# unknownue/puflow

Measured on AMD Instinct MI355X. Metric: patches/sec x4 2048->8192 (PU1K discrete, eval), higher is better.
Workload: dtype f32 (split-fp16 MFMA products, fp32 accumulate); 1 GPU; BASELINE configs[1]: PU1K discrete x4 inference, 32 x 2048-pt patches per GPU (fp32-parity mode); patches_per_gpu=32, total_batch=32, npoint=2048

## Files before the change

### include/puflow_hip.h

```cpp
#ifndef PUFLOW_HIP_H
#define PUFLOW_HIP_H

#ifdef __cplusplus
extern "C" {
#endif

#define PF_OK 0
#define PF_ERR_NULL (-1)
#define PF_ERR_SHAPE (-2)
#define PF_ERR_UNSUPPORTED (-3)
#define PF_ERR_LAUNCH (-4)
#define PF_ERR_WORKSPACE (-5)

int pf_version(void);
const char* pf_error_string(int code);

int pf_knn(const float* p1, const float* p2, int B, int N, int M, int K, int* idx_out, float* dist_out, void* stream);

int pf_nn1(const float* p1, const float* p2, int B, int N, int M, float* dist_out, int* idx_out, void* stream);

int pf_edgeconv(int cfg, const float* pq_or_xyz, const float* tab, const int* idx, const float* wfrag, float* out,
                int B, int N, void* stream);

int pf_edgeconv_tuned(int cfg, int variant, const float* pq_or_xyz, const float* tab, const int* idx,
                      const float* wfrag, float* out, int B, int N, void* stream);

int pf_edgeconv_pq(int unit, const float* pq_or_xyz, const int* idx, const float* wfrag, float* out, const float* w,
                   const long long* off, float* pq_next, int B, int N, int fuse, void* stream);

int pf_pq_gemm(int unit, const float* h, const float* w, const long long* off, float* pq_next, int T, void* stream);
int pf_cond(int unit, const float* h, const float* w, const long long* off, float* c, float* st, float* cp, int T,
            void* stream);
int pf_post(int unit, const float* h, const float* w, const long long* off, float* c, float* st, float* cp,
            float* pq_next, int T, void* stream);
int pf_cond_all(const float* const* h, const float* w, const long long* off, float* const* c, float* st, float* cp, int T,
                void* stream);

int pf_flow_fwd(const float* xyz, const float* cp, const float* st, const float* w, float* z, float* ld_pt, int T,
                void* stream);

int pf_flow_inv(const float* u, const float* cp, const float* st, const float* w, float* x, int T, int R, void* stream);

int pf_logp(const float* z, const float* ld_pt, float ld_const, int B, int N, float* ldj, float* lpsum, float* logp,
            void* stream);

long long pf_flow_fwd_logp_ws_floats(int B, int N);
int pf_flow_fwd_logp(const float* xyz, const float* cp, const float* st, const float* w, float* z, float* ld_pt,
                     float ld_const, int B, int N, float* ldj, float* lpsum, float* logp, float* ws, void* stream);

int pf_interp(const float* xyz, const float* z, const int* idx16, const float* w, const long long* off, float* u_out,
              int B, int N, int R, void* stream);

int pf_interp_weights(const float* xyz, const int* idx16, const float* w, const long long* off, float* aw_out, int B, int N,
                      void* stream);
int pf_flow_inv_interp(const float* aw, const float* z, const int* idx16, const float* cp, const float* st, const float* w,
                       float* x, int B, int N, int R, void* stream);

int pf_chamfer_fwd(const float* x, const float* y, int B, int N, int M, float* dist1, int* idx1, float* dist2,
                   int* idx2, float* per_sample, float* mean_sum, void* stream);

int pf_chamfer_bwd(const float* x, const float* y, const int* idx1, const int* idx2, const float* g1, const float* g2,
                   float* gx, float* gy, int B, int N, int M, void* stream);
int pf_chamfer_bwd_det(const float* x, const float* y, const int* idx1, const int* idx2, const float* g1, const float* g2,
                       float* gx, float* gy, int B, int N, int M, void* stream);

int pf_emd_forward(const float* xyz1, const float* xyz2, float* dist, int* assignment, float* price,
                   int* assignment_inv, int* bid, float* bid_increments, float* max_increments, int* unass_idx,
                   int* max_idx, float eps, int iters, int B, int n, void* stream);

int pf_emd_forward_ex(const float* xyz1, const float* xyz2, float* dist, int* assignment, float* price,
                      int* assignment_inv, int* bid, float* bid_increments, float* max_increments, int* unass_idx,
                      int* max_idx, float eps, int iters, int B, int n, int groups, unsigned* status, void* stream);

int pf_emd_backward(const float* xyz1, const float* xyz2, float* gradxyz, const float* graddist, const int* idx, int B,
                    int n, void* stream);


long long pf_gemm_ws_floats(int M, int N, int K);
int pf_gemm(const float* A, long long sam, long long sak, const float* B, long long sbk, long long sbn, float* C,
            long long ldc, const float* bias, int M, int N, int K, float* ws, long long ws_floats, void* stream);
int pf_gemm_reduce(const float* slabs, float* C, int M, int N, long long ldc, int nslab, void* stream);
int pf_gemm_ex(int arith, const float* A, long long sam, long long sak, const float* B, long long sbk, long long sbn, float* C,
               long long ldc, const float* bias, int M, int N, int K, float* ws, long long ws_floats, void* stream);

int pf_bn_chunks(long long R);
int pf_bn_lrelu_fwd(const float* x, long long R, int C, const float* gamma, const float* beta, float slope, float eps,
                    float momentum, float* run_mean, float* run_var, float* y, float* save, float* ws, void* stream);
int pf_bn_lrelu_bwd(const float* x, const float* dy, long long R, int C, const float* gamma, const float* beta, float slope,
                    const float* save, float* dx, float* dgamma, float* dbeta, float* ws, void* stream);
int pf_bn_colstat(const float* x, long long R, int C, const float* mean_in, float* out, float* ws, void* stream);
int pf_bn_apply_stats(const float* x, long long R, int C, const float* mean, const float* var_b, float unbias,
                      const float* gamma, const float* beta, float slope, float eps, float momentum, float* run_mean,
                      float* run_var, float* y, float* save, void* stream);
int pf_bn_bwd_sums(const float* x, const float* dy, long long R, int C, const float* gamma, const float* beta, float slope,
                   const float* save, float* sums, float* ws, void* stream);
int pf_bn_bwd_apply(const float* x, const float* dy, long long R, int C, const float* gamma, const float* beta, float slope,
                    const float* save, const float* means, float* dx, void* stream);
int pf_colsum(const float* g, long long R, int C, float* out, float* ws, void* stream);

int pf_act_fwd(const float* x, float slope, long long total, float* y, void* stream);
int pf_act_bwd(const float* y, const float* dy, float slope, long long total, float* dx, void* stream);

int pf_edge_feature_fwd(const float* x, const int* idx, int B, int N, int K, int C, float* out, void* stream);
int pf_edge_feature_bwd(const float* g, const int* idx, int B, int N, int K, int C, float* dx, void* stream);

int pf_maxpool_k_fwd(const float* y, long long T, int K, int C, float* out, int* arg, void* stream);
int pf_maxpool_k_bwd(const float* dy, const int* arg, long long T, int K, int C, float* dx, void* stream);

int pf_scatter_rows(const float* g, const int* idx, int B, int N, int K, int C, float* out, void* stream);
int pf_scatter_rows_det(const float* g, const int* csr_off, const int* csr_edge, long long T, int C, float* out, void* stream);
int pf_group_sum(const float* g, long long T, int R, int C, float* out, void* stream);

int pf_softmax_wsum_fwd(const float* w, int ldw, const float* zj, int K, int R, long long T, float* a, float* fz,
                        void* stream);
int pf_softmax_wsum_bwd(const float* a, const float* zj, const float* dfz, int K, int R, int ldw, long long T, float* dw,
                        float* dzj, void* stream);

int pf_actnorm_fwd(const float* x, const float* logs, const float* bias, int inv, long long R, float* y, void* stream);
int pf_actnorm_bwd(const float* x, const float* dy, const float* logs, const float* bias, int inv, long long R, float* dx,
                   float* glogs_rows, float* gbias_rows, void* stream);
int pf_couple_inject_fwd(const float* y, const float* o, const float* s, const float* t, int td, long long R, float* out,
                         void* stream);
int pf_couple_inject_bwd(const float* out, const float* dout, const float* s, int td, long long R, float* dy, float* do_,
                         float* ds, float* dt, void* stream);
int pf_inject_inv_fwd(const float* u, const float* s, const float* t, long long R, float* v, void* stream);
int pf_inject_inv_bwd(const float* u, const float* s, const float* dv, long long R, float* du, float* ds, float* dt,
                      void* stream);
int pf_couple_add(const float* v, const float* o, int td, long long R, float* out, void* stream);
int pf_slice_tail(const float* g, int td, long long R, float* o, void* stream);
int pf_batch_sum_fwd(const float* x, int B, long long M, int mode, float* out, void* stream);
int pf_batch_sum_bwd(const float* x, const float* g, int B, long long M, int mode, float* dx, void* stream);
int pf_dist_feature(const float* xyz, const int* idx, int B, int N, int K, float* out, void* stream);

#define PF_TRAIN_STAT_DOUBLES 4097
typedef struct PfEcTrain {
    int B, N, K, C, growth, nconv, odim, pooling;
    float slope, eps, momentum;
    const float* x;
    const int* idx;
    const float* W[9];
    const float* bias[9];
    const float* gamma[8]; const float* beta[8];
    float* run_mean[8]; float* run_var[8];
    float* Wpq;
    float* bpq;
    float* PQ;
    float* Y;
    float* aff;
    float* out;
    unsigned char* arg;
    const float* dout;
    float* dA;
    float* dPQ;
    float* coef;
    float* dWpq;
    float* dx;
    float* dW[9]; float* dbias[9]; float* dgamma[8]; float* dbeta[8];
    float* ws; long long ws_floats;
    double* stat;
    const int* csr_off; const int* csr_edge;
    int flags;
    unsigned* sync;
    int (*sync_cb)(void* user, double* sums, int n, void* stream);
    void* sync_user;
    double* sync_sums;
    float* ws_dw; long long ws_dw_floats;
    const float* dx_add;
} PfEcTrain;
#define PF_EC_PERSISTENT 1
#define PF_TRAIN_DETERMINISTIC 2
#define PF_EC_PREFOLDED 4
int pf_train_set_dw_stream(void* stream);
int pf_knn_csr(const int* idx, int B, int N, int K, int* off, int* edge, int* cnt, void* stream);
int pf_knn_csr_pair(const int* idx, int B, int N, int K, int K2, int* off, int* edge, int* off2, int* edge2, int* cnt, void* stream);

int pf_knn_csr_sort(const int* off, int* edge, int T, void* stream);
long long pf_ec_train_ws_floats(const PfEcTrain* p);
int pf_ec_train_fwd(const PfEcTrain* p, void* stream);
int pf_ec_train_fold_batch(const PfEcTrain* descs, int n, void* stream);
int pf_ec_train_bwd(const PfEcTrain* p, void* stream);

typedef struct PfBnMlpTrain {
    int rows, nl, kin0a, kin0b;
    int width[3];
    float slope, eps, momentum;
    const float* xa; const float* xb;
    const float* W[3]; const float* b[3];
// ... 287 lines not shown
```

### puflow_amd/_lib.py

```python
from __future__ import annotations

import ctypes
import os
from ctypes import c_char_p, c_double, c_float, c_int, c_longlong, c_ulonglong, c_void_p, POINTER

_HERE = os.path.dirname(os.path.abspath(__file__))
LIB_PATH = os.environ.get("PF_LIB_PATH", os.path.join(_HERE, "libpuflow_hip.so"))
_lib = None

class PfEcTrain(ctypes.Structure):
    _fields_ = [("B", c_int), ("N", c_int), ("K", c_int), ("C", c_int), ("growth", c_int), ("nconv", c_int), ("odim", c_int),
                ("pooling", c_int), ("slope", c_float), ("eps", c_float), ("momentum", c_float),
                ("x", c_void_p), ("idx", c_void_p), ("W", c_void_p * 9), ("bias", c_void_p * 9),
                ("gamma", c_void_p * 8), ("beta", c_void_p * 8), ("run_mean", c_void_p * 8), ("run_var", c_void_p * 8),
                ("Wpq", c_void_p), ("bpq", c_void_p), ("PQ", c_void_p), ("Y", c_void_p), ("aff", c_void_p), ("out", c_void_p),
                ("arg", c_void_p), ("dout", c_void_p), ("dA", c_void_p), ("dPQ", c_void_p), ("coef", c_void_p),
                ("dWpq", c_void_p), ("dx", c_void_p), ("dW", c_void_p * 9), ("dbias", c_void_p * 9),
                ("dgamma", c_void_p * 8), ("dbeta", c_void_p * 8), ("ws", c_void_p), ("ws_floats", c_longlong), ("stat", c_void_p), ("csr_off", c_void_p), ("csr_edge", c_void_p),
                ("flags", c_int), ("sync", c_void_p), ("sync_cb", c_void_p), ("sync_user", c_void_p), ("sync_sums", c_void_p),
                ("ws_dw", c_void_p), ("ws_dw_floats", c_longlong), ("dx_add", c_void_p)]


class PfBnMlpTrain(ctypes.Structure):
    _fields_ = [("rows", c_int), ("nl", c_int), ("kin0a", c_int), ("kin0b", c_int), ("width", c_int * 3),
                ("slope", c_float), ("eps", c_float), ("momentum", c_float), ("xa", c_void_p), ("xb", c_void_p),
                ("W", c_void_p * 3), ("b", c_void_p * 3), ("gamma", c_void_p * 2), ("beta", c_void_p * 2),
                ("run_mean", c_void_p * 2), ("run_var", c_void_p * 2), ("y", c_void_p * 3), ("aff", c_void_p * 2),
                ("dout", c_void_p), ("d", c_void_p * 2), ("coef", c_void_p * 2), ("dxa", c_void_p), ("dxb", c_void_p),
                ("dW", c_void_p * 3), ("db", c_void_p * 3), ("dgamma", c_void_p * 2), ("dbeta", c_void_p * 2),
                ("ws", c_void_p), ("ws_floats", c_longlong), ("stat", c_void_p),
                ("sync_cb", c_void_p), ("sync_user", c_void_p), ("sync_sums", c_void_p), ("flags", c_int)]


class PfMlpTrain(ctypes.Structure):
    _fields_ = [("rows", c_int), ("nl", c_int), ("td", c_int), ("ldy", c_int), ("cc", c_int), ("cdiv", c_int),
                ("width", c_int * 3), ("slope", c_float * 2), ("y", c_void_p), ("c", c_void_p),
                ("W", c_void_p * 3), ("b", c_void_p * 3), ("h", c_void_p * 2), ("out", c_void_p), ("dout", c_void_p),
                ("dz", c_void_p * 2), ("dy", c_void_p), ("dc", c_void_p), ("dW", c_void_p * 3), ("db", c_void_p * 3),
                ("ws", c_void_p), ("ws_floats", c_longlong), ("chunk", c_int), ("flags", c_int)]


_P8 = c_void_p * 8


class PfFlowChain(ctypes.Structure):
    _fields_ = [("nb", c_int), ("rows", c_int), ("R", c_int), ("inv", c_int), ("td", c_int * 8), ("cc", c_int * 8), ("n_ld", c_float),
                ("x", c_void_p), ("c", _P8), ("s", _P8), ("t", _P8), ("logs", _P8), ("bias", _P8), ("W", _P8),
                ("w0", _P8), ("w2", _P8), ("b2", _P8), ("w4", _P8), ("b4", _P8),
                ("pin", c_void_p), ("mid", c_void_p), ("o", c_void_p), ("h1", c_void_p), ("h2", c_void_p), ("out", c_void_p),
                ("ssum", c_void_p), ("ld", c_void_p), ("logp", c_void_p), ("Bsz", c_int), ("part", c_void_p), ("counter", c_void_p), ("img", c_void_p),
                ("dout", c_void_p), ("dssum", c_void_p), ("dld", c_void_p), ("dlogp", c_void_p), ("dx", c_void_p),
                ("dc", _P8), ("ds", _P8), ("dt", _P8), ("dz1", c_void_p), ("dz2", c_void_p), ("dob", c_void_p),
                ("dlogs", _P8), ("dbias", _P8), ("dW", _P8), ("dw0", _P8), ("dw2", _P8), ("db2", _P8), ("dw4", _P8), ("db4", _P8),
                ("ws", c_void_p), ("ws_floats", c_longlong), ("dev_descs", c_void_p), ("dz1s", c_void_p), ("img_ready", c_int)]


class PfPoissonPool(ctypes.Structure):
    _fields_ = [("off", c_int), ("s", c_int), ("m", c_int), ("out_off", c_int), ("R2", c_float), ("inv", c_float), ("lo", c_float),
                ("path", c_int)]


SIGNATURES = {
    "pf_version": (c_int, []),
    "pf_error_string": (c_char_p, [c_int]),
    "pf_knn": (c_int, [c_void_p, c_void_p, c_int, c_int, c_int, c_int, c_void_p, c_void_p, c_void_p]),
    "pf_nn1": (c_int, [c_void_p, c_void_p, c_int, c_int, c_int, c_void_p, c_void_p, c_void_p]),
    "pf_edgeconv": (c_int, [c_int, c_void_p, c_void_p, c_void_p, c_void_p, c_void_p, c_int, c_int, c_void_p]),
    "pf_edgeconv_tuned": (c_int, [c_int, c_int, c_void_p, c_void_p, c_void_p, c_void_p, c_void_p, c_int, c_int,
                                  c_void_p]),
    "pf_edgeconv_pq": (c_int, [c_int, c_void_p, c_void_p, c_void_p, c_void_p, c_void_p, POINTER(c_longlong), c_void_p, c_int, c_int, c_int,
                               c_void_p]),
    "pf_post": (c_int, [c_int, c_void_p, c_void_p, POINTER(c_longlong), c_void_p, c_void_p, c_void_p, c_void_p, c_int,
                        c_void_p]),
    "pf_pq_gemm": (c_int, [c_int, c_void_p, c_void_p, POINTER(c_longlong), c_void_p, c_int, c_void_p]),
    "pf_cond_all": (c_int, [POINTER(c_void_p), c_void_p, POINTER(c_longlong), POINTER(c_void_p), c_void_p, c_void_p, c_int, c_void_p]),
    "pf_cond": (c_int, [c_int, c_void_p, c_void_p, POINTER(c_longlong), c_void_p, c_void_p, c_void_p, c_int, c_void_p]),
    "pf_flow_fwd": (c_int, [c_void_p, c_void_p, c_void_p, c_void_p, c_void_p, c_void_p, c_int, c_void_p]),
    "pf_flow_inv": (c_int, [c_void_p, c_void_p, c_void_p, c_void_p, c_void_p, c_int, c_int, c_void_p]),
    "pf_flow_fwd_logp_ws_floats": (c_longlong, [c_int, c_int]),
    "pf_flow_fwd_logp": (c_int, [c_void_p, c_void_p, c_void_p, c_void_p, c_void_p, c_void_p, c_float, c_int, c_int, c_void_p, c_void_p,
                                 c_void_p, c_void_p, c_void_p]),
    "pf_logp": (c_int, [c_void_p, c_void_p, c_float, c_int, c_int, c_void_p, c_void_p, c_void_p, c_void_p]),
    "pf_interp": (c_int, [c_void_p, c_void_p, c_void_p, c_void_p, POINTER(c_longlong), c_void_p, c_int, c_int, c_int,
                          c_void_p]),
    "pf_interp_weights": (c_int, [c_void_p, c_void_p, c_void_p, POINTER(c_longlong), c_void_p, c_int, c_int, c_void_p]),
    "pf_flow_inv_interp": (c_int, [c_void_p, c_void_p, c_void_p, c_void_p, c_void_p, c_void_p, c_void_p, c_int, c_int, c_int, c_void_p]),
    "pf_chamfer_fwd": (c_int, [c_void_p, c_void_p, c_int, c_int, c_int, c_void_p, c_void_p, c_void_p, c_void_p, c_void_p,
                               c_void_p, c_void_p]),
    "pf_chamfer_bwd": (c_int, [c_void_p, c_void_p, c_void_p, c_void_p, c_void_p, c_void_p, c_void_p, c_void_p, c_int,
                               c_int, c_int, c_void_p]),
    "pf_chamfer_bwd_det": (c_int, [c_void_p, c_void_p, c_void_p, c_void_p, c_void_p, c_void_p, c_void_p, c_void_p, c_int,
                                   c_int, c_int, c_void_p]),
    "pf_emd_forward": (c_int, [c_void_p] * 11 + [c_float, c_int, c_int, c_int, c_void_p]),
    "pf_emd_forward_ex": (c_int, [c_void_p] * 11 + [c_float, c_int, c_int, c_int, c_int, c_void_p, c_void_p]),
    "pf_emd_backward": (c_int, [c_void_p, c_void_p, c_void_p, c_void_p, c_void_p, c_int, c_int, c_void_p]),
    "pf_gemm_ws_floats": (c_longlong, [c_int, c_int, c_int]),
    "pf_gemm": (c_int, [c_void_p, c_longlong, c_longlong, c_void_p, c_longlong, c_longlong, c_void_p, c_longlong, c_void_p,
                        c_int, c_int, c_int, c_void_p, c_longlong, c_void_p]),
    "pf_gemm_reduce": (c_int, [c_void_p, c_void_p, c_int, c_int, c_longlong, c_int, c_void_p]),
    "pf_gemm_ex": (c_int, [c_int, c_void_p, c_longlong, c_longlong, c_void_p, c_longlong, c_longlong, c_void_p, c_longlong, c_void_p,
                        c_int, c_int, c_int, c_void_p, c_longlong, c_void_p]),
    "pf_bn_chunks": (c_int, [c_longlong]),
    "pf_bn_lrelu_fwd": (c_int, [c_void_p, c_longlong, c_int, c_void_p, c_void_p, c_float, c_float, c_float, c_void_p,
                                c_void_p, c_void_p, c_void_p, c_void_p, c_void_p]),
    "pf_bn_lrelu_bwd": (c_int, [c_void_p, c_void_p, c_longlong, c_int, c_void_p, c_void_p, c_float, c_void_p, c_void_p,
                                c_void_p, c_void_p, c_void_p, c_void_p]),
    "pf_bn_colstat": (c_int, [c_void_p, c_longlong, c_int, c_void_p, c_void_p, c_void_p, c_void_p]),
    "pf_bn_apply_stats": (c_int, [c_void_p, c_longlong, c_int, c_void_p, c_void_p, c_float, c_void_p, c_void_p, c_float, c_float,
                                  c_float, c_void_p, c_void_p, c_void_p, c_void_p, c_void_p]),
    "pf_bn_bwd_sums": (c_int, [c_void_p, c_void_p, c_longlong, c_int, c_void_p, c_void_p, c_float, c_void_p, c_void_p, c_void_p,
                               c_void_p]),
    "pf_bn_bwd_apply": (c_int, [c_void_p, c_void_p, c_longlong, c_int, c_void_p, c_void_p, c_float, c_void_p, c_void_p, c_void_p,
                                c_void_p]),
    "pf_colsum": (c_int, [c_void_p, c_longlong, c_int, c_void_p, c_void_p, c_void_p]),
    "pf_act_fwd": (c_int, [c_void_p, c_float, c_longlong, c_void_p, c_void_p]),
    "pf_act_bwd": (c_int, [c_void_p, c_void_p, c_float, c_longlong, c_void_p, c_void_p]),
    "pf_edge_feature_fwd": (c_int, [c_void_p, c_void_p, c_int, c_int, c_int, c_int, c_void_p, c_void_p]),
    "pf_edge_feature_bwd": (c_int, [c_void_p, c_void_p, c_int, c_int, c_int, c_int, c_void_p, c_void_p]),
    "pf_maxpool_k_fwd": (c_int, [c_void_p, c_longlong, c_int, c_int, c_void_p, c_void_p, c_void_p]),
    "pf_maxpool_k_bwd": (c_int, [c_void_p, c_void_p, c_longlong, c_int, c_int, c_void_p, c_void_p]),
    "pf_scatter_rows": (c_int, [c_void_p, c_void_p, c_int, c_int, c_int, c_int, c_void_p, c_void_p]),
    "pf_scatter_rows_det": (c_int, [c_void_p, c_void_p, c_void_p, c_longlong, c_int, c_void_p, c_void_p]),
    "pf_group_sum": (c_int, [c_void_p, c_longlong, c_int, c_int, c_void_p, c_void_p]),
    "pf_softmax_wsum_fwd": (c_int, [c_void_p, c_int, c_void_p, c_int, c_int, c_longlong, c_void_p, c_void_p, c_void_p]),
    "pf_softmax_wsum_bwd": (c_int, [c_void_p, c_void_p, c_void_p, c_int, c_int, c_int, c_longlong, c_void_p, c_void_p,
                                    c_void_p]),
    "pf_actnorm_fwd": (c_int, [c_void_p, c_void_p, c_void_p, c_int, c_longlong, c_void_p, c_void_p]),
    "pf_actnorm_bwd": (c_int, [c_void_p, c_void_p, c_void_p, c_void_p, c_int, c_longlong, c_void_p, c_void_p, c_void_p, c_void_p]),
    "pf_couple_inject_fwd": (c_int, [c_void_p, c_void_p, c_void_p, c_void_p, c_int, c_longlong, c_void_p, c_void_p]),
    "pf_couple_inject_bwd": (c_int, [c_void_p, c_void_p, c_void_p, c_int, c_longlong, c_void_p, c_void_p, c_void_p, c_void_p,
                                     c_void_p]),
    "pf_inject_inv_fwd": (c_int, [c_void_p, c_void_p, c_void_p, c_longlong, c_void_p, c_void_p]),
    "pf_inject_inv_bwd": (c_int, [c_void_p, c_void_p, c_void_p, c_longlong, c_void_p, c_void_p, c_void_p, c_void_p]),
    "pf_couple_add": (c_int, [c_void_p, c_void_p, c_int, c_longlong, c_void_p, c_void_p]),
    "pf_slice_tail": (c_int, [c_void_p, c_int, c_longlong, c_void_p, c_void_p]),
    "pf_batch_sum_fwd": (c_int, [c_void_p, c_int, c_longlong, c_int, c_void_p, c_void_p]),
    "pf_batch_sum_bwd": (c_int, [c_void_p, c_void_p, c_int, c_longlong, c_int, c_void_p, c_void_p]),
    "pf_dist_feature": (c_int, [c_void_p, c_void_p, c_int, c_int, c_int, c_void_p, c_void_p]),
    "pf_fps": (c_int, [c_void_p, c_int, c_int, c_int, c_void_p, c_void_p, c_void_p]),
    "pf_fps_grouped": (c_int, [c_void_p, c_int, c_int, c_int, c_int, c_void_p, c_void_p, c_void_p]),
    "pf_fps_scratch_layout": (c_int, [c_int, POINTER(c_longlong), POINTER(c_longlong)]),
    "pf_fps_exchange_probe": (c_int, [c_int, c_int, c_void_p, c_void_p]),
    "pf_flow_params_fwd": (c_int, [c_void_p, c_void_p, c_float, c_void_p, c_void_p, c_void_p]),
    "pf_flow_params_bwd": (c_int, [c_void_p, c_void_p, c_void_p, c_float, c_void_p, c_void_p, c_void_p]),
    "pf_flow_affine_fwd": (c_int, [c_void_p, c_void_p, c_int, c_void_p, c_void_p, c_void_p, c_int, c_longlong, c_void_p, c_void_p]),
    "pf_flow_affine_bwd": (c_int, [c_void_p, c_void_p, c_int, c_void_p, c_void_p, c_void_p, c_int, c_longlong, c_void_p, c_void_p,
                                   c_void_p, c_void_p, c_void_p, c_void_p, c_void_p, c_void_p, c_void_p]),
    "pf_couple_inject2_fwd": (c_int, [c_void_p, c_void_p, c_void_p, c_void_p, c_int, c_longlong, c_void_p, c_void_p, c_void_p,
                                      c_void_p, c_void_p]),
    "pf_couple_inject2_bwd": (c_int, [c_void_p, c_void_p, c_void_p, c_void_p, c_int, c_longlong, c_void_p, c_void_p, c_void_p,
                                      c_void_p, c_void_p]),
    "pf_inject_inv2_fwd": (c_int, [c_void_p, c_void_p, c_void_p, c_int, c_longlong, c_void_p, c_void_p]),
    "pf_inject_inv2_bwd": (c_int, [c_void_p, c_void_p, c_void_p, c_int, c_longlong, c_void_p, c_void_p, c_void_p, c_void_p]),
    "pf_clip_adam": (c_int, [c_void_p, c_void_p, c_void_p, c_void_p, c_void_p, c_int, c_void_p, c_void_p, c_float, c_float, c_float,
                             c_float, c_void_p, c_void_p, c_void_p, c_void_p]),
    "pf_clip_adam_ptrs": (c_int, [c_void_p, c_void_p, c_void_p, c_void_p, c_void_p, c_int, c_void_p, c_void_p, c_float, c_float, c_float,
                             c_float, c_void_p, c_void_p, c_void_p, c_void_p]),
    "pf_mlp_train_ws_floats": (c_longlong, [c_void_p]),
    "pf_mlp_train_fwd": (c_int, [c_void_p, c_void_p]),
    "pf_mlp_train_bwd": (c_int, [c_void_p, c_void_p]),
    "pf_mlp_train_fwd_batch": (c_int, [c_void_p, c_int, c_void_p, c_void_p]),
    "pf_mlp_train_bwd_batch": (c_int, [c_void_p, c_int, c_void_p, c_void_p]),
    "pf_mlp_train_dw_batch": (c_int, [c_void_p, c_int, c_void_p, c_void_p]),
    "pf_flowchain_ws_floats": (c_longlong, [c_void_p]),
    "pf_flowchain_part_floats": (c_longlong, [c_void_p]),
    "pf_flowchain_img_floats": (c_longlong, [c_void_p]),
    "pf_flowchain_fwd": (c_int, [c_void_p, c_void_p]),
    "pf_flowchain_bwd": (c_int, [c_void_p, c_void_p]),
    "pf_interp_wsum_fwd": (c_int, [c_void_p, c_int, c_void_p, c_void_p, c_int, c_int, c_int, c_longlong, c_void_p, c_void_p, c_void_p]),
    "pf_interp_wsum_bwd": (c_int, [c_void_p, c_void_p, c_void_p, c_void_p, c_int, c_int, c_int, c_int, c_longlong, c_void_p, c_void_p,
                                   c_void_p]),
    "pf_interp_wsum_bwd_det": (c_int, [c_void_p, c_void_p, c_void_p, c_void_p, c_int, c_int, c_int, c_int, c_longlong, c_void_p, c_void_p,
                                       c_void_p, c_void_p, c_void_p]),
    "pf_emd_init": (c_int, [c_void_p, c_void_p, c_longlong, c_void_p]),
    "pf_pugan_loss_fwd": (c_int, [c_void_p, c_void_p, c_void_p, c_void_p, c_int, c_int, c_float, c_float, c_float, c_void_p, c_void_p]),
    "pf_pugan_loss_bwd": (c_int, [c_void_p, c_void_p, c_int, c_int, c_int, c_float, c_float, c_float, c_void_p, c_void_p, c_void_p,
                                  c_void_p, c_void_p, c_void_p, c_void_p]),
    "pf_pugan_grad": (c_int, [c_void_p] * 7 + [c_int] * 3 + [c_float] * 3 + [c_void_p] * 3),
    "pf_bnmlp_train_ws_floats": (c_longlong, [c_void_p]),
    "pf_bnmlp_train_fwd": (c_int, [c_void_p, c_void_p]),
    "pf_bnmlp_train_bwd": (c_int, [c_void_p, c_void_p]),
    "pf_train_set_dw_stream": (c_int, [c_void_p]),
    "pf_fold_wu_fwd": (c_int, [c_void_p] * 6 + [c_int] * 3 + [c_void_p] * 5),
    "pf_fold_wu_bwd": (c_int, [c_void_p] * 5 + [c_int] * 3 + [c_void_p] * 11),
    "pf_knn_csr": (c_int, [c_void_p, c_int, c_int, c_int, c_void_p, c_void_p, c_void_p, c_void_p]),
    "pf_knn_csr_pair": (c_int, [c_void_p, c_int, c_int, c_int, c_int, c_void_p, c_void_p, c_void_p, c_void_p, c_void_p, c_void_p]),
    "pf_knn_csr_sort": (c_int, [c_void_p, c_void_p, c_int, c_void_p]),
    "pf_ec_train_ws_floats": (c_longlong, [c_void_p]),
    "pf_ec_train_fwd": (c_int, [c_void_p, c_void_p]),
    "pf_ec_train_fold_batch": (c_int, [c_void_p, c_int, c_void_p]),
    "pf_ec_train_bwd": (c_int, [c_void_p, c_void_p]),
    "pf_cnf_init": (c_int, [c_void_p, c_void_p, c_int, c_void_p, c_void_p, c_void_p, c_void_p, c_void_p, c_double, c_double, c_double,
                            c_void_p, c_double, c_int, c_float, c_float, c_int, c_int, c_void_p, c_void_p]),
    "pf_cnf_context": (c_int, [c_void_p, c_int, c_void_p, c_void_p, c_float, c_void_p, c_int, c_void_p]),
    "pf_cnf_steps": (c_int, [c_void_p, c_void_p, c_void_p, c_void_p, c_void_p, c_void_p, c_void_p, c_void_p, c_void_p, c_float,
                             c_float, c_int, c_int, c_int, c_void_p, c_int, c_void_p]),
    "pf_knn_large": (c_int, [c_void_p, c_void_p, c_int, c_int, c_int, c_int, c_void_p, c_void_p, c_void_p]),
    "pf_normalize_pc": (c_int, [c_void_p, c_int, c_int, c_void_p, c_void_p, c_void_p, c_void_p]),
    "pf_normalize_pc_ragged": (c_int, [c_void_p, POINTER(c_int), c_int, c_void_p, c_void_p, c_void_p, c_void_p]),
    "pf_fps_ragged_layout": (c_int, [POINTER(c_int), c_int, c_int, POINTER(c_longlong), POINTER(c_int), POINTER(c_longlong),
                                     POINTER(c_longlong), POINTER(c_longlong)]),
    "pf_fps_ragged": (c_int, [c_void_p, POINTER(c_int), POINTER(c_int), c_int, c_int, c_void_p, c_void_p, c_void_p]),
    "pf_knn_large_ragged": (c_int, [c_void_p, c_void_p, POINTER(c_int), POINTER(c_int), c_int, c_int, c_void_p, c_void_p, c_void_p]),
    "pf_nn1_ragged": (c_int, [c_void_p, c_void_p, POINTER(c_int), POINTER(c_int), c_int, c_void_p, c_void_p, c_void_p]),
    "pf_format_xyz_bound": (c_longlong, [c_longlong, c_int]),
    "pf_format_xyz": (c_longlong, [c_void_p, c_longlong, c_int, c_void_p, c_longlong]),
    "pf_parse_xyz": (c_longlong, [c_void_p, c_longlong, c_void_p, c_longlong, POINTER(c_int)]),
    "pf_cnf_rhs": (c_int, [c_void_p, c_void_p, POINTER(c_float), c_int, c_float, c_float, c_float, c_void_p, c_void_p,
                           c_void_p, c_void_p, c_void_p, c_int, c_int, c_void_p]),
    "pf_cnf_rhs_vjp_workspace_bytes": (c_longlong, [c_int, c_int]),
    "pf_cnf_rhs_vjp": (c_int, [c_void_p, c_void_p, c_float, c_float, c_void_p, c_void_p, c_void_p, c_void_p, c_void_p, c_void_p,
                               c_int, c_int, c_void_p, c_void_p]),
    "pf_cnf_step": (c_int, [c_void_p, c_void_p, c_float, c_float, c_int, c_void_p, c_void_p, c_void_p, c_void_p, c_void_p,
                            c_void_p, c_float, c_float, c_int, c_int, c_void_p, c_void_p, c_void_p]),
    "pf_sum_n": (c_int, [POINTER(c_void_p), c_int, c_void_p, c_longlong, c_void_p]),
    "pf_copy_n": (c_int, [POINTER(c_void_p), POINTER(c_void_p), POINTER(c_longlong), c_int, c_void_p]),
    "pf_lincomb": (c_int, [POINTER(c_void_p), POINTER(c_float), c_int, c_void_p, c_longlong, c_void_p]),
    "pf_scaled_sumsq": (c_int, [c_void_p, c_void_p, c_void_p, c_void_p, c_void_p, POINTER(c_float), c_int, c_float, c_float,
                                c_float, c_longlong, c_void_p, c_void_p, c_void_p]),
    "pf_approxmatch_ws_floats": (c_longlong, [c_int, c_int, c_int, c_int]),
    "pf_approxmatch_emd": (c_int, [c_void_p, c_void_p, c_int, c_int, c_int, c_int, c_void_p, c_void_p, c_longlong, c_void_p]),
    "pf_point_mesh_ws_floats": (c_longlong, [c_int, c_int]),
    "pf_point_mesh_dist": (c_int, [c_void_p, c_int, c_void_p, c_int, c_void_p, c_int, c_void_p, c_void_p, c_void_p, c_longlong,
                                   c_void_p]),
    "pf_patch_batch": (c_int, [c_void_p, c_void_p, c_void_p, c_void_p, c_int, c_int, c_int, c_longlong, c_int, c_int, c_ulonglong,
                               c_ulonglong, c_int, c_float, c_float, c_float, c_float, c_float, c_void_p, c_void_p, c_void_p,
                               c_void_p, c_void_p, c_void_p, c_int, c_void_p, c_void_p]),
# ... 64 lines not shown
```

### puflow_amd/build.py

```python
from __future__ import annotations

import os
import subprocess
import sys

HERE = os.path.dirname(os.path.abspath(__file__))
CSRC = os.path.join(HERE, "csrc")
LIB = os.path.join(HERE, "libpuflow_hip.so")
SOURCES = ["api.hip", "knn.hip", "edgeconv.hip", "pointwise.hip", "flow.hip", "interp.hip", "chamfer.hip", "emd.hip", "train_ops.hip", "train_fused.hip", "train_ec_fwd.hip", "train_csr.hip", "train_bnmlp.hip", "train_mlp.hip", "train_flow.hip", "train_flowchain.hip", "train_glue.hip", "optim.hip", "patch_ops.hip", "cnf.hip", "cnf_bwd.hip", "xyz_io.hip", "eval_metrics.hip", "data_aug.hip", "eval_uniform.hip", "poisson.hip", "surface_reach.hip"]
FLAGS = ["--offload-arch=gfx950", "-O3", "-std=c++17", "-fPIC", "-ffp-contract=on", "-Wno-unused-result"]
EXTRA_FLAGS = {s: ["-fno-honor-nans", "-mllvm", "-amdgpu-mfma-vgpr-form=" + os.environ.get("PF_MFMA_VGPR_FORM", "1")] for s in ("edgeconv.hip", "pointwise.hip", "flow.hip", "interp.hip", "cnf.hip", "cnf_bwd.hip")}
EXTRA_FLAGS["edgeconv.hip"] = EXTRA_FLAGS["edgeconv.hip"] + ["-DPF_W2LDS_DEPTH=" + os.environ.get("PF_EC_W2LDS_DEPTH", "3")]
if os.environ.get("PF_INTERP_TRACKERS", "1") != "0":
    EXTRA_FLAGS["interp.hip"] = EXTRA_FLAGS["interp.hip"] + ["-mllvm", "-amdgpu-use-amdgpu-trackers=1"]


def _stale(target: str, deps) -> bool:
    if not os.path.exists(target):
        return True
    t = os.path.getmtime(target)
    return any(os.path.getmtime(d) > t for d in deps)


F16_SOURCES = ("edgeconv.hip", "pointwise.hip", "flow.hip", "interp.hip")
LIB_F16 = LIB.replace(".so", "_f16.so")


def build(force: bool = False, verbose: bool = True, defines=(), tag: str = "", only=None) -> str:
    hipcc = os.environ.get("HIPCC", "/opt/rocm/bin/hipcc")
    lib = LIB if not tag else LIB.replace(".so", f"_{tag}.so")
    srcs = [os.path.join(CSRC, s) for s in SOURCES if os.path.exists(os.path.join(CSRC, s))]
    hdrs = [os.path.join(CSRC, h) for h in os.listdir(CSRC) if h.endswith(".h")]
    hdrs.append(os.path.join(os.path.dirname(HERE), "include", "puflow_hip.h"))
    objdir = os.path.join(HERE, "build" + (f"_{tag}" if tag else ""))
    maindir = os.path.join(HERE, "build")
    os.makedirs(objdir, exist_ok=True)
    objs = []
    procs = []
    for s in srcs:
        base = os.path.basename(s)
        if only is not None and base not in only:
            objs.append(os.path.join(maindir, base.replace(".hip", ".o")))
            continue
        o = os.path.join(objdir, base.replace(".hip", ".o"))
        objs.append(o)
        if force or _stale(o, [s] + hdrs):
            cmd = [hipcc] + FLAGS + EXTRA_FLAGS.get(os.path.basename(s), []) + [f"-D{d}" for d in defines] + ["-c", s, "-o", o]
            if verbose:
                print(" ".join(cmd), flush=True)
            procs.append((s, subprocess.Popen(cmd)))
    for s, p in procs:
        if p.wait() != 0:
            raise RuntimeError(f"hipcc failed on {s}")
    if force or procs or _stale(lib, objs):
        cmd = [hipcc, "--offload-arch=gfx950", "-shared", "-fPIC", "-o", lib] + objs
        if verbose:
            print(" ".join(cmd), flush=True)
        subprocess.check_call(cmd)
    global _REFRESHING
    if not tag and not defines and not _REFRESHING:
        _REFRESHING = True
        try:
            _refresh_variants(lib, verbose)
        finally:
            _REFRESHING = False
    return lib


_REFRESHING = False


def _refresh_variants(lib: str, verbose: bool) -> None:
    pkg = os.path.dirname(lib)
    if os.path.exists(os.path.join(pkg, "libpuflow_hip_f16.so")) and _stale(os.path.join(pkg, "libpuflow_hip_f16.so"), [lib]):
        build_f16(verbose=verbose)
    if any(os.path.exists(os.path.join(pkg, f"libpuflow_hip_{t}.so")) and _stale(os.path.join(pkg, f"libpuflow_hip_{t}.so"), [lib])
           for t in ("bwdf32", "gradf32")):
        build_gradf32(verbose=verbose)


def build_f16(force: bool = False, verbose: bool = True) -> str:
    build(force=False, verbose=verbose)
    return build(force=force, verbose=verbose, defines=["PF_MMN_TERMS=1"], tag="f16", only=F16_SOURCES)


LIB_GRADF32 = LIB.replace(".so", "_gradf32.so")
GRADF32_DEFINES = ["PF_EC_BWDG_F32", "PF_EC_DW_F32", "PF_EC_FWD_F32"]
LIB_BWDF32 = LIB.replace(".so", "_bwdf32.so")
BWDF32_DEFINES = ["PF_EC_BWDG_F32", "PF_EC_DW_F32"]


def build_gradf32(force: bool = False, verbose: bool = True) -> str:
    build(force=False, verbose=verbose)
    build(force=force, verbose=verbose, defines=BWDF32_DEFINES, tag="bwdf32", only=("train_fused.hip",))
    return build(force=force, verbose=verbose, defines=GRADF32_DEFINES, tag="gradf32", only=("train_fused.hip", "train_ec_fwd.hip"))


if __name__ == "__main__":
    build(force="--force" in sys.argv)
    build_f16(force="--force" in sys.argv)
    build_gradf32(force="--force" in sys.argv)
    print(LIB)
    print(LIB_F16)
    print(LIB_GRADF32)
```

### puflow_amd/csrc/edgeconv.hip

```cpp
#include <hip/hip_runtime.h>
#include "pf_api_internal.h"
#include "pf_mfma.h"

namespace {

struct EcArgs {
    const float* pq;
    const float* xyz;
    const float* tab;
    const int* idx;
    const f4* wg;
    float* out;
    int T;
    int N;
    int chunk;
    int ntiles;
    const u4* pqf_w;
    const float* pqf_bias;
    const float* pqf_scales;
    float* pqf_out;
};

template <int ODIM>
__device__ __forceinline__ void pqf_stage(u4* hb, int ch, int pt, float v) {
    _Float16* h = reinterpret_cast<_Float16*>(hb);
    const int cp = ch >> 5, j = ((ch >> 4) & 1) * 4 + (ch & 3), slot = 16 * ((ch & 15) >> 2) + pt;
    const _Float16 hi = (_Float16)v;
    const _Float16 lo = (_Float16)(v - (float)hi);
    h[((cp * 2 + 0) * 64 + slot) * 8 + j] = hi;
    h[((cp * 2 + 1) * 64 + slot) * 8 + j] = lo;
}

constexpr int PQF_NT = 4;

template <int ODIM, int ROWS, int NW>
__device__ __forceinline__ void pqf_gemm(const EcArgs& a, const u4* hb, int nst, const int (&tpt)[PQF_NT], int wave_u, int lane) {
    constexpr int CP = ODIM / 32, RB = ROWS / 16 / NW;
    static_assert(ODIM % 32 == 0 && ROWS % (16 * NW) == 0, "rows split evenly over the waves");
    constexpr int OBW = NW <= 8 ? RB : 1;
    const int col = lane & 15, q = lane >> 4;
    const PfW2BufD<CP> ws(a.pqf_w, lane);
    const float inv = a.pqf_scales[6];
#pragma unroll
    for (int ob0 = 0; ob0 < RB; ob0 += OBW) {
        h8 wh[OBW][CP], wl[OBW][CP];
#pragma unroll
        for (int o = 0; o < OBW; ++o)
#pragma unroll
            for (int cp = 0; cp < CP; ++cp) {
                wh[o][cp] = ws.load((wave_u * RB + ob0 + o) * CP + cp, 0);
                wl[o][cp] = ws.load((wave_u * RB + ob0 + o) * CP + cp, 1);
            }
#pragma unroll
        for (int t = 0; t < PQF_NT; ++t) {
            if (t >= nst) break;
            const u4* hbt = hb + t * (CP * 2 * 64);
            f4 acc[OBW];
#pragma unroll
            for (int o = 0; o < OBW; ++o) acc[o] = pf_splat(0.f);
#pragma unroll
            for (int cp = 0; cp < CP; ++cp) {
                const h8 fh = __builtin_bit_cast(h8, hbt[(cp * 2 + 0) * 64 + lane]), fl = __builtin_bit_cast(h8, hbt[(cp * 2 + 1) * 64 + lane]);
#pragma unroll
                for (int o = 0; o < OBW; ++o) {
                    f4 x = acc[o];
                    if constexpr (PF_MMN_TERMS == 3) {
                        x = pf_mfma_f16(wh[o][cp], fl, x);
                        x = pf_mfma_f16(wl[o][cp], fh, x);
                    }
                    x = pf_mfma_f16(wh[o][cp], fh, x);
                    acc[o] = x;
                }
            }
            const int pt = tpt[t] + col;
            if (pt < a.T) {
#pragma unroll
                for (int o = 0; o < OBW; ++o) {
                    const f4 bias = *reinterpret_cast<const f4*>(a.pqf_bias + (wave_u * RB + ob0 + o) * 16 + 4 * q);
                    f4 v;
#pragma unroll
                    for (int r = 0; r < 4; ++r) v[r] = fmaf(acc[o][r], inv, bias[r]);
                    *reinterpret_cast<f4*>(a.pqf_out + (size_t)pt * ROWS + (wave_u * RB + ob0 + o) * 16 + 4 * q) = v;
                }
            }
        }
    }
}

struct PqfState {
    int nst = 0;
    int tpt[PQF_NT] = {0, 0, 0, 0};
    __device__ __forceinline__ void push(int pt0) {
#pragma unroll
        for (int k = 0; k < PQF_NT; ++k) tpt[k] = k == nst ? pt0 : tpt[k];
        ++nst;
    }
};

template <int GB, int NCONV, int ODIM, bool C3, int P, int NW>
__global__ __launch_bounds__(NW * 64) void edgeconv_kernel(EcArgs a) {
    constexpr int G = GB * 16;
    constexpr int S = G * NCONV + ODIM;
    constexpr int NF = GB * NCONV;
    constexpr int OBO = ODIM / 16;
    constexpr int OCH = 2;
    static_assert(OBO <= 16 && OBO % OCH == 0, "pooled store uses one lane column per output block");
    const int lane = threadIdx.x & 63, wave = threadIdx.x >> 6;
    const int col = lane & 15, q = lane >> 4;

    constexpr int NWF = GB * GB * (NCONV * (NCONV - 1) / 2) + OBO * NF;
    __shared__ f4 wlds[NWF * 64];
    pf_stage_lds(wlds, a.wg, NWF * 64);
    __syncthreads();
    const PfWLds ws{wlds, lane};

    for (int v = blockIdx.x; v < 8 * a.chunk; v += gridDim.x) {
        const int tile = pf_xcd_tile(v, a.chunk);
        if (tile >= a.ntiles) continue;
        const int pt0 = (tile * NW + wave) * P;

        int gi[P], gj[P];
        float xi[P][3], xj[P][3];
#pragma unroll
        for (int p = 0; p < P; ++p) {
            int g = pt0 + p;
            g = g < a.T ? g : a.T - 1;
            gi[p] = g;
            const int b = g / a.N;
            gj[p] = b * a.N + a.idx[(size_t)g * 16 + col];
            if constexpr (C3) {
#pragma unroll
                for (int c = 0; c < 3; ++c) {
                    xi[p][c] = a.xyz[(size_t)gi[p] * 3 + c];
                    xj[p][c] = a.xyz[(size_t)gj[p] * 3 + c];
                }
            }
        }

        auto init = [&](int p, int off) -> f4 {
            if constexpr (C3) {
                f4 r;
#pragma unroll
                for (int k = 0; k < 4; ++k) {
                    const f4* t = reinterpret_cast<const f4*>(a.tab + (size_t)(off + k) * 8);
                    const f4 t0 = t[0], t1 = t[1];
                    float s = t1.z;
                    s = fmaf(t0.x, xi[p][0], s); s = fmaf(t0.y, xi[p][1], s); s = fmaf(t0.z, xi[p][2], s);
                    s = fmaf(t0.w, xj[p][0], s); s = fmaf(t1.x, xj[p][1], s); s = fmaf(t1.y, xj[p][2], s);
                    r[k] = s;
                }
                return r;
            } else {
                const f4 pv = *reinterpret_cast<const f4*>(a.pq + (size_t)gi[p] * (2 * S) + off);
                const f4 qv = *reinterpret_cast<const f4*>(a.pq + (size_t)gj[p] * (2 * S) + S + off);
                return pv + qv;
            }
        };

        constexpr int NI = GB > OCH ? GB : OCH;
        f4 ini[2][P][NI];
        auto load_init = [&](auto nbc, int row0, f4 (&dst)[P][NI]) {
            constexpr int NB = decltype(nbc)::value;
#pragma unroll
            for (int ob = 0; ob < NB; ++ob)
#pragma unroll
                for (int p = 0; p < P; ++p) dst[p][ob] = init(p, row0 + ob * 16 + 4 * q);
        };
        using IGB = std::integral_constant<int, GB>;
        using IOC = std::integral_constant<int, OCH>;
        load_init(IGB{}, 0, ini[0]);
        if constexpr (NCONV > 1) load_init(IGB{}, G, ini[1]); else load_init(IOC{}, G * NCONV, ini[1]);

        f4 feat[P][NF];
#pragma unroll
        for (int ob = 0; ob < GB; ++ob)
#pragma unroll
            for (int p = 0; p < P; ++p) feat[p][ob] = pf_lrelu(ini[0][p][ob], 0.05f);

        pf_static_for<1, NCONV>([&](auto tc) {
            constexpr int t = decltype(tc)::value;
            if constexpr (t + 1 < NCONV) load_init(IGB{}, G * (t + 1), ini[(t + 1) & 1]);
            else load_init(IOC{}, G * NCONV, ini[(t + 1) & 1]);
            f4 acc[P][GB];
#pragma unroll
            for (int ob = 0; ob < GB; ++ob)
#pragma unroll
                for (int p = 0; p < P; ++p) acc[p][ob] = ini[t & 1][p][ob];
            pf_mm<GB, GB * t, GB * t>(ws, GB * GB * (t * (t - 1) / 2), feat, 0, acc, 0);
#pragma unroll
            for (int ob = 0; ob < GB; ++ob)
#pragma unroll
                for (int p = 0; p < P; ++p) feat[p][GB * t + ob] = pf_lrelu(acc[p][ob], 0.05f);
        });

        constexpr int FO = GB * GB * (NCONV * (NCONV - 1) / 2);
        f4 sel[P];
#pragma unroll
        for (int p = 0; p < P; ++p) sel[p] = pf_splat(0.f);
        pf_static_for<0, OBO / OCH>([&](auto cc) {
            constexpr int c = decltype(cc)::value;
            constexpr int ob0 = c * OCH;
            constexpr int st = NCONV + c;
            if constexpr (c + 1 < OBO / OCH) load_init(IOC{}, G * NCONV + (ob0 + OCH) * 16, ini[(st + 1) & 1]);
            f4 acc[P][OCH];
#pragma unroll
            for (int o = 0; o < OCH; ++o)
#pragma unroll
                for (int p = 0; p < P; ++p) acc[p][o] = ini[st & 1][p][o];
            pf_mm<OCH, NF, NF>(ws, FO + ob0 * NF, feat, 0, acc, 0);
#pragma unroll
            for (int o = 0; o < OCH; ++o)
#pragma unroll
                for (int p = 0; p < P; ++p) {
                    f4 m;
#pragma unroll
                    for (int r = 0; r < 4; ++r) m[r] = pf_rowmax16(acc[p][o][r]);
                    if (col == ob0 + o) sel[p] = m;
                }
        });
#pragma unroll
        for (int p = 0; p < P; ++p)
            if (col < OBO && pt0 + p < a.T)
                *reinterpret_cast<f4*>(a.out + (size_t)gi[p] * ODIM + col * 16 + 4 * q) = sel[p];
    }
}

struct EcWConst {
    static constexpr int DEPTH = 2;
    int lane;
    __device__ __forceinline__ h8 load(int frag, int split) const {
        const _Float16 x = (_Float16)(float)((lane + frag + split) & 7);
        return (h8){x, x, x, x, x, x, x, x};
    }
};

constexpr float EC4_OUT_INV = 1.f / 256.f;

template <int P, int NW, int DBG = 0, bool PQF = false>
__global__ __launch_bounds__(NW * 64) void edgeconv4_kernel(EcArgs a) {
    static_assert(!PQF || NW * P == 16, "the fused P|Q GEMM takes a workgroup tile of 16 points as one MFMA column tile");
    constexpr int NCONV = 4, G = 32, S = 256, OBO = 8, OCH = 2, ODIM = 128;
    constexpr int NWF = 2 * (NCONV * (NCONV - 1) / 2) + OBO * NCONV;
    constexpr int ROWB = 2 * S * 4;
    const int lane = threadIdx.x & 63, wave = threadIdx.x >> 6;
    const int col = lane & 15, q = lane >> 4;
    __shared__ u4 wlds[NWF * 2 * 64];
    __shared__ f4 plds[NW * P][64];
    __shared__ u4 hb[PQF ? PQF_NT * (ODIM / 32) * 2 * 64 : 1];
    PqfState pqf;
    pf_stage_lds(wlds, reinterpret_cast<const u4*>(a.wg), NWF * 2 * 64);
    __syncthreads();
    const PfW2Lds ws_lds{wlds, lane};
    const auto ws = [&] { if constexpr ((DBG & 4) != 0) return EcWConst{lane}; else return ws_lds; }();
    const __amdgpu_buffer_rsrc_t rs = __builtin_amdgcn_make_buffer_rsrc(const_cast<float*>(a.pq), 0, 0x7fffffff, 0x00020000);
    const int blkq = ((q & 1) << 1) | (q >> 1);

    const int vend = 8 * a.chunk;
    auto next_valid = [&](int v) { while (v < vend && pf_xcd_tile(v, a.chunk) >= a.ntiles) v += gridDim.x; return v; };
    struct Pre { int g[P]; int jc[P]; int4 j4[P]; f4 prow[P]; };
    auto fetch = [&](int v, Pre& n) {
        const int pt0 = (pf_xcd_tile(v < vend ? v : blockIdx.x, a.chunk) * NW + wave) * P;
#pragma unroll
        for (int p = 0; p < P; ++p) {
            int g = pt0 + p;
            g = g < a.T ? g : a.T - 1;
            g = __builtin_amdgcn_readfirstlane(g);
            n.g[p] = g;
            n.jc[p] = a.idx[(size_t)g * 16 + col];
            n.j4[p] = *reinterpret_cast<const int4*>(a.idx + (size_t)g * 16 + 4 * q);
            n.prow[p] = __builtin_bit_cast(f4, __builtin_amdgcn_raw_buffer_load_b128(rs, lane * 16, g * ROWB, 0));
        }
    };
    int v = next_valid(blockIdx.x);
    Pre cur;
    if (v < vend) fetch(v, cur);
    while (v < vend) {
        const int pt0 = (pf_xcd_tile(v, a.chunk) * NW + wave) * P;
        const int vn = next_valid(v + gridDim.x);
        int vQ[P];
        int vO[P][4];
        int gout[P];
#pragma unroll
        for (int p = 0; p < P; ++p) {
            const int g = cur.g[p];
            const int bN = (g / a.N) * a.N;
            gout[p] = g;
            plds[wave * P + p][lane] = cur.prow[p];
            vQ[p] = (bN + cur.jc[p]) * ROWB + (S + 4 * q) * 4;
            vO[p][0] = (bN + cur.j4[p].x) * ROWB + (S + G * NCONV + col) * 4;
            vO[p][1] = (bN + cur.j4[p].y) * ROWB + (S + G * NCONV + col) * 4;
            vO[p][2] = (bN + cur.j4[p].z) * ROWB + (S + G * NCONV + col) * 4;
            vO[p][3] = (bN + cur.j4[p].w) * ROWB + (S + G * NCONV + col) * 4;
        }
        fetch(vn, cur);
        auto load_g = [&](int t, f4 (&dst)[P][2]) {
#pragma unroll
            for (int ob = 0; ob < 2; ++ob)
#pragma unroll
                for (int p = 0; p < P; ++p) {
                    const int off = (G * t + 16 * ob) * 4;
                    if constexpr (DBG & 1) { dst[p][ob] = pf_splat((float)(off + vQ[p]) * 1e-9f); continue; }
                    dst[p][ob] = __builtin_bit_cast(f4, __builtin_amdgcn_raw_buffer_load_b128(rs, vQ[p], off, 0));
                }
        };
        auto p_g = [&](int p, int t, int ob) -> f4 { return plds[wave * P + p][(G * t + 16 * ob) / 4 + q]; };
        auto load_o = [&](int ob0, f4 (&dst)[P][2]) {
#pragma unroll
            for (int o = 0; o < OCH; ++o)
#pragma unroll
                for (int p = 0; p < P; ++p)
#pragma unroll
                    for (int r = 0; r < 4; ++r) {
                        if constexpr (DBG & 1) { dst[p][o][r] = (float)(vO[p][r] + ob0 + o) * 1e-9f; continue; }
                        dst[p][o][r] = __builtin_bit_cast(float, __builtin_amdgcn_raw_buffer_load_b32(rs, vO[p][r], (ob0 + o) * 64, 0));
                    }
        };
        f4 ini[2][P][2];
        load_g(0, ini[0]);
        load_g(1, ini[1]);
        PfPairN feat[P][NCONV];
#pragma unroll
        for (int p = 0; p < P; ++p)
            feat[p][0] = pf_pairn(pf_lrelu(ini[0][p][0] + p_g(p, 0, 0), 0.05f), pf_lrelu(ini[0][p][1] + p_g(p, 0, 1), 0.05f));
        pf_static_for<1, NCONV>([&](auto tc) {
            constexpr int t = decltype(tc)::value;
            if constexpr (t + 1 < NCONV) load_g(t + 1, ini[(t + 1) & 1]); else load_o(0, ini[(t + 1) & 1]);
            f4 acc[P][2];
#pragma unroll
            for (int ob = 0; ob < 2; ++ob)
#pragma unroll
                for (int p = 0; p < P; ++p) acc[p][ob] = ini[t & 1][p][ob] + p_g(p, t, ob);
            if constexpr (!(DBG & 2)) pf_mmn<false, 2, t, t>(ws, 2 * (t * (t - 1) / 2), feat, acc);
#pragma unroll
            for (int p = 0; p < P; ++p) {
                if constexpr (DBG & 8) { feat[p][t] = feat[p][0]; feat[p][t].h[0] += (_Float16)acc[p][0].x; continue; }
                feat[p][t] = pf_pairn(pf_lrelu(acc[p][0], 0.05f), pf_lrelu(acc[p][1], 0.05f));
            }
        });
        constexpr int FO = 2 * (NCONV * (NCONV - 1) / 2);
        float m[P][OBO];
        pf_static_for<0, OBO / OCH>([&](auto cc) {
            constexpr int c = decltype(cc)::value;
            constexpr int ob0 = c * OCH;
            constexpr int st = NCONV + c;
            if constexpr (c + 1 < OBO / OCH) load_o(ob0 + OCH, ini[(st + 1) & 1]);
            f4 acc[P][OCH];
#pragma unroll
            for (int o = 0; o < OCH; ++o)
#pragma unroll
                for (int p = 0; p < P; ++p) acc[p][o] = ini[st & 1][p][o];
            if constexpr (!(DBG & 2)) pf_mmn<true, OCH, NCONV, NCONV>(ws, FO + ob0 * NCONV, feat, acc);
#pragma unroll
            for (int o = 0; o < OCH; ++o)
#pragma unroll
                for (int p = 0; p < P; ++p)
                    m[p][ob0 + o] = fmaxf(fmaxf(acc[p][o].x, acc[p][o].y), fmaxf(acc[p][o].z, acc[p][o].w));
        });
#pragma unroll
        for (int p = 0; p < P; ++p) {
            const float o0 = pf_rsmax16(pf_rsmax32(m[p][0], m[p][1]), pf_rsmax32(m[p][2], m[p][3]));
            const float o1 = pf_rsmax16(pf_rsmax32(m[p][4], m[p][5]), pf_rsmax32(m[p][6], m[p][7]));
            const int ch = 16 * blkq + col;
            const float* pr = reinterpret_cast<const float*>(plds[wave * P + p]);
            const float p0 = pr[G * NCONV + ch], p1 = pr[G * NCONV + 64 + ch];
            const float h0 = fmaf(o0, EC4_OUT_INV, p0), h1 = fmaf(o1, EC4_OUT_INV, p1);
            if (pt0 + p < a.T) {
                float* o = a.out + (size_t)gout[p] * ODIM + ch;
                o[0] = h0;
                o[64] = h1;
            }
            if constexpr (PQF) {
                u4* hbt = hb + pqf.nst * ((ODIM / 32) * 2 * 64);
                pqf_stage<ODIM>(hbt, ch, wave * P + p, h0);
                pqf_stage<ODIM>(hbt, ch + 64, wave * P + p, h1);
            }
        }
        if constexpr (PQF) {
            pqf.push(pf_xcd_tile(v, a.chunk) * NW * P);
            if (pqf.nst == PQF_NT || vn >= vend) {
                __syncthreads();
                pqf_gemm<ODIM, 2 * S, NW>(a, hb, pqf.nst, pqf.tpt, __builtin_amdgcn_readfirstlane(wave), lane);
                __syncthreads();
                pqf.nst = 0;
            }
        }
        v = vn;
    }
}

template <int P, int NW, int DBG = 0, bool PQF = false>
int launch4(const EcArgs& a0, hipStream_t s) {
    EcArgs a = a0;
    a.ntiles = (a.T + NW * P - 1) / (NW * P);
    a.chunk = (a.ntiles + 7) / 8;
    int grid = 8 * a.chunk;
    if (grid > 256) grid = 256;
    hipLaunchKernelGGL((edgeconv4_kernel<P, NW, DBG, PQF>), dim3(grid), dim3(NW * 64), 0, s, a);
    return pf_last_launch_status();
}

template <int ODIM, bool C3, int P, int NW, bool PQF = false>
__global__ __launch_bounds__(NW * 64) void edgeconv1n_kernel(EcArgs a) {
    static_assert(!PQF || NW * P == 16, "the fused P|Q GEMM takes a workgroup tile of 16 points as one MFMA column tile");
    constexpr int NCONV = 4, S = 16 * NCONV + ODIM, SB = S / 16, OBO = ODIM / 16;
    constexpr int PQ_ROWS = ODIM == 32 ? 256 : 512;
    constexpr int FO = 4, FT = FO + OBO * 2, NWF = FT + (C3 ? SB : 0);
    constexpr int ROWB = 2 * S * 4;
    static_assert(OBO == 2 || OBO == 4, "reduce-scatter below is written for 2 or 4 output blocks");
    const int lane = threadIdx.x & 63, wave = threadIdx.x >> 6;
    const int col = lane & 15, q = lane >> 4;
    __shared__ u4 wlds[NWF * 128];
    __shared__ float plds[C3 ? 1 : NW * P][C3 ? 1 : S];
    __shared__ u4 hb[PQF ? PQF_NT * (ODIM / 32) * 2 * 64 : 1];
    PqfState pqf;
    pf_stage_lds(wlds, reinterpret_cast<const u4*>(a.wg), NWF * 128);
    __syncthreads();
    const PfW2Lds ws{wlds, lane};
    const __amdgpu_buffer_rsrc_t rs = __builtin_amdgcn_make_buffer_rsrc(const_cast<float*>(C3 ? a.xyz : a.pq), 0, 0x7fffffff, 0x00020000);

    for (int v = blockIdx.x; v < 8 * a.chunk; v += gridDim.x) {
        const int tile = pf_xcd_tile(v, a.chunk);
        if (tile >= a.ntiles) continue;
        const int pt0 = (tile * NW + wave) * P;
        int gi[P], vQ[P], vO[P][4];
        PfPairN e[P][1];
#pragma unroll
        for (int p = 0; p < P; ++p) {
            int g = pt0 + p;
            g = g < a.T ? g : a.T - 1;
            g = __builtin_amdgcn_readfirstlane(g);
            gi[p] = g;
            const int bN = (g / a.N) * a.N;
            const int jc = bN + a.idx[(size_t)g * 16 + col];
            if constexpr (C3) {
                float xi[3], xj[3];
#pragma unroll
                for (int c = 0; c < 3; ++c) {
                    xi[c] = a.xyz[(size_t)g * 3 + c];
                    xj[c] = a.xyz[(size_t)jc * 3 + c];
                }
                const f4 z4 = pf_splat(0.f);
                const f4 e0 = {xi[0], xi[1], xi[2], xj[0]}, e1 = {xj[1], xj[2], 0.f, 1.f};
                e[p][0] = pf_pairn(q == 0 ? e0 : z4, q == 0 ? e1 : z4);
            } else {
                const int4 j4 = *reinterpret_cast<const int4*>(a.idx + (size_t)g * 16 + 4 * q);
                vQ[p] = jc * ROWB + (S + 4 * q) * 4;
                vO[p][0] = (bN + j4.x) * ROWB + (S + 16 * NCONV + col) * 4;
                vO[p][1] = (bN + j4.y) * ROWB + (S + 16 * NCONV + col) * 4;
                vO[p][2] = (bN + j4.z) * ROWB + (S + 16 * NCONV + col) * 4;
                vO[p][3] = (bN + j4.w) * ROWB + (S + 16 * NCONV + col) * 4;
                if (lane * 2 < S) {
                    typedef float f2 __attribute__((ext_vector_type(2)));
                    const f2 pv = *reinterpret_cast<const f2*>(a.pq + (size_t)g * (2 * S) + lane * 2);
                    *reinterpret_cast<f2*>(&plds[wave * P + p][lane * 2]) = pv;
                }
            }
        }
        f4 pre[P][NCONV];
        f4 outi[P][OBO];
        if constexpr (C3) {
#pragma unroll
            for (int p = 0; p < P; ++p) {
#pragma unroll
                for (int b = 0; b < NCONV; ++b) pre[p][b] = pf_splat(0.f);
#pragma unroll
                for (int b = 0; b < OBO; ++b) outi[p][b] = pf_splat(0.f);
            }
            pf_mmn<false, NCONV, 1, 1>(ws, FT, e, pre);
            pf_mmn<true, OBO, 1, 1>(ws, FT + NCONV, e, outi);
        } else {
#pragma unroll
            for (int b = 0; b < NCONV; ++b)
#pragma unroll
                for (int p = 0; p < P; ++p)
                    pre[p][b] = __builtin_bit_cast(f4, __builtin_amdgcn_raw_buffer_load_b128(rs, vQ[p], b * 64, 0));
#pragma unroll
            for (int b = 0; b < OBO; ++b)
#pragma unroll
                for (int p = 0; p < P; ++p)
#pragma unroll
                    for (int r = 0; r < 4; ++r)
                        outi[p][b][r] = __builtin_bit_cast(float, __builtin_amdgcn_raw_buffer_load_b32(rs, vO[p][r], b * 64, 0));
#pragma unroll
            for (int b = 0; b < NCONV; ++b)
#pragma unroll
                for (int p = 0; p < P; ++p) pre[p][b] += *reinterpret_cast<const f4*>(&plds[wave * P + p][16 * b + 4 * q]);
        }

        PfPairN fp[P][2];
        f4 last[P];
#pragma unroll
        for (int p = 0; p < P; ++p) {
            last[p] = pf_lrelu(pre[p][0], 0.05f);
            fp[p][0] = pf_pairn(last[p], pf_splat(0.f));
        }
        pf_static_for<1, NCONV>([&](auto tc) {
            constexpr int t = decltype(tc)::value;
            constexpr int CPT = (t + 1) / 2, F0 = (t / 2) * ((t + 1) / 2);
            f4 acc[P][1];
#pragma unroll
            for (int p = 0; p < P; ++p) acc[p][0] = pre[p][t];
            pf_mmn<false, 1, CPT, CPT>(ws, F0, fp, acc);
#pragma unroll
            for (int p = 0; p < P; ++p) {
                const f4 f = pf_lrelu(acc[p][0], 0.05f);
                if constexpr (t % 2 == 1) fp[p][t / 2] = pf_pairn(last[p], f);
                else fp[p][t / 2] = pf_pairn(f, pf_splat(0.f));
                last[p] = f;
            }
        });
        pf_mmn<true, OBO, 2, 2>(ws, FO, fp, outi);
#pragma unroll
        for (int p = 0; p < P; ++p) {
            float m[OBO];
#pragma unroll
            for (int b = 0; b < OBO; ++b) m[b] = fmaxf(fmaxf(outi[p][b].x, outi[p][b].y), fmaxf(outi[p][b].z, outi[p][b].w));
            float o;
            int ch;
            if constexpr (OBO == 4) {
                o = pf_rsmax16(pf_rsmax32(m[0], m[1]), pf_rsmax32(m[2], m[3]));
                ch = 16 * (((q & 1) << 1) | (q >> 1)) + col;
            } else {
                const float n = pf_rsmax32(m[0], m[1]);
                o = pf_rsmax16(n, n);
                ch = 16 * (q >> 1) + col;
            }
            float pv = 0.f;
            if constexpr (!C3) pv = plds[wave * P + p][16 * NCONV + ch];
            const float hv = fmaf(o, EC4_OUT_INV, pv);
            if (pt0 + p < a.T && (OBO == 4 || (q & 1) == 0))
                a.out[(size_t)gi[p] * ODIM + ch] = hv;
            if constexpr (PQF) {
                if (OBO == 4 || (q & 1) == 0) pqf_stage<ODIM>(hb + pqf.nst * ((ODIM / 32) * 2 * 64), ch, wave * P + p, hv);
            }
        }
        if constexpr (PQF) {
            pqf.push(tile * NW * P);
            if (pqf.nst == PQF_NT) {
                __syncthreads();
                pqf_gemm<ODIM, PQ_ROWS, NW>(a, hb, pqf.nst, pqf.tpt, __builtin_amdgcn_readfirstlane(wave), lane);
                __syncthreads();
                pqf.nst = 0;
            }
        }
    }
    if constexpr (PQF) {
        if (pqf.nst > 0) {
            __syncthreads();
            pqf_gemm<ODIM, PQ_ROWS, NW>(a, hb, pqf.nst, pqf.tpt, __builtin_amdgcn_readfirstlane(wave), lane);
        }
    }
}

template <int ODIM, bool C3, int P, int NW, bool PQF = false>
int launch1n(const EcArgs& a0, hipStream_t s) {
    EcArgs a = a0;
    a.ntiles = (a.T + NW * P - 1) / (NW * P);
    a.chunk = (a.ntiles + 7) / 8;
    int grid = 8 * a.chunk;
    const int cap = 256 * (32 / NW);
    if (grid > cap) grid = cap;
    hipLaunchKernelGGL((edgeconv1n_kernel<ODIM, C3, P, NW, PQF>), dim3(grid), dim3(NW * 64), 0, s, a);
    return pf_last_launch_status();
}

template <int ODIM, bool C3>
int launch1n_v(const EcArgs& a, hipStream_t s, int variant) {
    switch (variant) {
        case 1: return launch1n<ODIM, C3, 2, 8>(a, s);
#ifdef PF_TUNING_VARIANTS
        case 0: return launch1n<ODIM, C3, 1, 8>(a, s);
        case 2: return launch1n<ODIM, C3, 1, 16>(a, s);
        case 3: return launch1n<ODIM, C3, 2, 4>(a, s);
#endif
        default: return PF_ERR_UNSUPPORTED;
    }
}

template <int GB, int NCONV, int ODIM, bool C3, int P, int NW>
int launch_v(const EcArgs& a0, hipStream_t s) {
    EcArgs a = a0;
    a.ntiles = (a.T + NW * P - 1) / (NW * P);
    a.chunk = (a.ntiles + 7) / 8;
    constexpr int NF = GB * NCONV;
    constexpr int lds = (GB * GB * (NCONV * (NCONV - 1) / 2) + (ODIM / 16) * NF) * 1024;
    int per_cu = (160 * 1024) / lds;
    const int by_waves = 32 / NW;
    if (per_cu > by_waves) per_cu = by_waves;
    if (per_cu < 1) per_cu = 1;
    int grid = 8 * a.chunk;
    const int cap = 256 * per_cu;
    if (grid > cap) grid = cap;
    hipLaunchKernelGGL((edgeconv_kernel<GB, NCONV, ODIM, C3, P, NW>), dim3(grid), dim3(NW * 64), 0, s, a);
    return pf_last_launch_status();
}

template <int GB, int NCONV, int ODIM, bool C3>
int launch(const EcArgs& a, hipStream_t s, int variant) {
    constexpr int BEST = ODIM == 32 ? 0 : (ODIM == 64 ? 2 : 3);
    if (variant == BEST) {
        if constexpr (BEST == 0) return launch_v<GB, NCONV, ODIM, C3, 2, 8>(a, s);
        else if constexpr (BEST == 2) return launch_v<GB, NCONV, ODIM, C3, 1, 8>(a, s);
        else return launch_v<GB, NCONV, ODIM, C3, 1, 16>(a, s);
    }
#ifdef PF_TUNING_VARIANTS
    switch (variant) {
        case 0: return launch_v<GB, NCONV, ODIM, C3, 2, 8>(a, s);
        case 1: return launch_v<GB, NCONV, ODIM, C3, 2, 4>(a, s);
        case 2: return launch_v<GB, NCONV, ODIM, C3, 1, 8>(a, s);
        case 3: return launch_v<GB, NCONV, ODIM, C3, 1, 16>(a, s);
        default: break;
    }
#endif
    return PF_ERR_UNSUPPORTED;
}

}

extern "C" int pf_edgeconv_tuned(int cfg, int variant, const float* pq_or_xyz, const float* tab, const int* idx,
                                 const float* wfrag, float* out, int B, int N, void* stream) {
    if (!pq_or_xyz || !idx || !wfrag || !out) return PF_ERR_NULL;
    if (B <= 0 || N < 16 || (long long)B * N > (1ll << 30)) return PF_ERR_SHAPE;
    EcArgs a{};
    a.idx = idx; a.wg = reinterpret_cast<const f4*>(wfrag); a.out = out; a.T = B * N; a.N = N;
    hipStream_t s = (hipStream_t)stream;
    switch (cfg) {
        case 0:
            if (!tab) return PF_ERR_NULL;
            a.xyz = pq_or_xyz; a.tab = tab;
            return launch<1, 4, 32, true>(a, s, variant);
        case 1: a.pq = pq_or_xyz; return launch<1, 4, 64, false>(a, s, variant);
        case 2: a.pq = pq_or_xyz; return launch<2, 4, 128, false>(a, s, variant);
        case 7:
            {
                const long long maxT = 0x7fffffffll / 2048;
                if (N > maxT) return PF_ERR_UNSUPPORTED;
                const int Bc = (int)(maxT / N);
                for (int b0 = 0; b0 < B; b0 += Bc) {
                    const int nb = B - b0 < Bc ? B - b0 : Bc;
                    EcArgs c = a;
                    c.pq = pq_or_xyz + (size_t)b0 * N * 512; c.idx = idx + (size_t)b0 * N * 16; c.out = out + (size_t)b0 * N * 128;
                    c.T = nb * N;
                    int rc;
                    switch (variant) {
                        case 0: rc = launch4<1, 16>(c, s); break;
#ifdef PF_TUNING_VARIANTS
                        case 1: rc = launch4<2, 8>(c, s); break;
                        case 2: rc = launch4<1, 8>(c, s); break;
                        case 3: rc = launch4<2, 4>(c, s); break;
                        case 8: rc = launch4<1, 16, 1>(c, s); break;
                        case 9: rc = launch4<1, 16, 2>(c, s); break;
                        case 10: rc = launch4<1, 16, 4>(c, s); break;
                        case 11: rc = launch4<1, 16, 5>(c, s); break;
                        case 12: rc = launch4<1, 16, 3>(c, s); break;
                        case 13: rc = launch4<1, 16, 6>(c, s); break;
                        case 14: rc = launch4<1, 16, 13>(c, s); break;
#endif
                        default: return PF_ERR_UNSUPPORTED;
                    }
                    if (rc != PF_OK) return rc;
// ... 47 lines not shown
```

### puflow_amd/csrc/flow.hip

```cpp
#include <hip/hip_runtime.h>
#include "pf_api_internal.h"
#include "pf_mfma.h"
#include "pf_wave.h"

#ifndef PF_FLOW_NW
#define PF_FLOW_NW 16
#endif
#ifndef PF_FLOW_NW_FWD
#define PF_FLOW_NW_FWD 16
#endif

namespace {

constexpr int FLOW_REC = 5360;
constexpr float LOG2PI_F = 1.8378770664093453f;

struct FlowArgs {
    const float* in;
    const float* cp;
    const float* st;
    const float* w;
    float* out;
    float* ld_pt;
    int T;
    int R;
    int rows;
    int ntiles;
    float* part;
    unsigned* counter;
    float* ldj; float* lps; float* logp;
    float ld_const;
    int B, N;
    const float* aw;
    const float* z;
    const int* idx;
};

struct FlowCond { f4 cp[4]; f4 s0, s1; };

__device__ __forceinline__ FlowCond flow_cond(const float* __restrict__ cp, const float* __restrict__ st, int T, int u,
                                              int pt, int q) {
    FlowCond c;
    const float* cr = cp + ((size_t)u * T + pt) * 64 + 4 * q;
#pragma unroll
    for (int cb = 0; cb < 4; ++cb) c.cp[cb] = *reinterpret_cast<const f4*>(cr + cb * 16);
    const float* sr = st + ((size_t)u * T + pt) * 8;
    c.s0 = *reinterpret_cast<const f4*>(sr);
    c.s1 = *reinterpret_cast<const f4*>(sr + 4);
    return c;
}

template <int TD>
__device__ __forceinline__ void coupling_net(const float* rec , int lane, int q, const FlowCond& c,
                                             const float (&h1)[2], float (&o)[2]) {
    PfPairN hp[1][2];
    const float i2 = rec[5352], i4 = rec[5353];
    {
        f4 hid[4];
#pragma unroll
        for (int cb = 0; cb < 4; ++cb) {
            const f4 wa = *reinterpret_cast<const f4*>(rec + 5200 + (cb * 16 + 4 * q) * 2);
            const f4 wb = *reinterpret_cast<const f4*>(rec + 5200 + (cb * 16 + 4 * q) * 2 + 4);
            f4 v = c.cp[cb];
            v.x = fmaf(wa.x, h1[0], v.x); v.y = fmaf(wa.z, h1[0], v.y);
            v.z = fmaf(wb.x, h1[0], v.z); v.w = fmaf(wb.z, h1[0], v.w);
            if (TD == 2) {
                v.x = fmaf(wa.y, h1[1], v.x); v.y = fmaf(wa.w, h1[1], v.y);
                v.z = fmaf(wb.y, h1[1], v.z); v.w = fmaf(wb.w, h1[1], v.w);
            }
            hid[cb] = pf_lrelu(v, 0.01f);
        }
        hp[0][0] = pf_pairn(hid[0], hid[1]);
        hp[0][1] = pf_pairn(hid[2], hid[3]);
    }
    const PfW2Lds ws{reinterpret_cast<const u4*>(rec), lane};
    f4 h2[1][4];
#pragma unroll
    for (int ob = 0; ob < 4; ++ob) h2[0][ob] = pf_bias(rec + 5120, ob, q);
    pf_mmn<false, 4, 2, 2>(ws, 0, hp, h2);
    hp[0][0] = pf_pairn(pf_lrelu(h2[0][0] * i2, 0.01f), pf_lrelu(h2[0][1] * i2, 0.01f));
    hp[0][1] = pf_pairn(pf_lrelu(h2[0][2] * i2, 0.01f), pf_lrelu(h2[0][3] * i2, 0.01f));
    f4 acc[1][1];
    acc[0][0] = *reinterpret_cast<const f4*>(rec + 5184 + 4 * q);
    pf_mmn<false, 1, 2, 2>(ws, 8, hp, acc);
    o[0] = acc[0][0].x * i4; o[1] = acc[0][0].y * i4;
}

template <bool INV, int NW>
__global__ __launch_bounds__(NW * 64) void flow_kernel(FlowArgs a) {
    const int lane = threadIdx.x & 63, wave = threadIdx.x >> 6;
    const int col = lane & 15, q = lane >> 4;
    __shared__ f4 wl[6 * FLOW_REC / 4];
    pf_stage_lds(wl, reinterpret_cast<const f4*>(a.w), 6 * FLOW_REC / 4);
    __syncthreads();
    const float* wlf = reinterpret_cast<const float*>(wl);

    for (int tile = blockIdx.x; tile < a.ntiles; tile += gridDim.x) {
        const int g = (tile * NW + wave) * 16 + col;
        const bool ok = g < a.rows;
        const int row = ok ? g : a.rows - 1;
        const int pt = row / a.R;
        float v[3], ld = 0.f;
        if (INV && a.aw) {
            const int r = row - pt * a.R, bN = (pt / a.N) * a.N;
            const int4 j0 = *reinterpret_cast<const int4*>(a.idx + (size_t)pt * 16), j1 = *reinterpret_cast<const int4*>(a.idx + (size_t)pt * 16 + 4);
            const int jj[8] = {j0.x, j0.y, j0.z, j0.w, j1.x, j1.y, j1.z, j1.w};
            float sk[8][3];
#pragma unroll
            for (int k = 0; k < 8; ++k) {
                const float wk = a.aw[((size_t)pt * 8 + k) * 4 + r];
                const float* zz = a.z + (size_t)(bN + jj[k]) * 3;
#pragma unroll
                for (int c = 0; c < 3; ++c) sk[k][c] = __fmul_rn(wk, zz[c]);
            }
#pragma unroll
            for (int c = 0; c < 3; ++c)
                v[c] = __fadd_rn(__fadd_rn(__fadd_rn(sk[0][c], sk[1][c]), __fadd_rn(sk[2][c], sk[3][c])),
                                 __fadd_rn(__fadd_rn(sk[4][c], sk[5][c]), __fadd_rn(sk[6][c], sk[7][c])));
        } else {
#pragma unroll
            for (int c = 0; c < 3; ++c) v[c] = a.in[(size_t)row * 3 + c];
        }
        FlowCond cn = flow_cond(a.cp, a.st, a.T, INV ? 5 : 0, pt, q);

        pf_static_for<0, 6>([&](auto uc) {
            constexpr int i = decltype(uc)::value;
            constexpr int u = INV ? 5 - i : i;
            constexpr int TD = (u % 2 == 0) ? 1 : 2;
            const float* rec = wlf + u * FLOW_REC;
            const float* fc = rec + 5328;
            const FlowCond c = cn;
            if constexpr (i < 5) cn = flow_cond(a.cp, a.st, a.T, INV ? u - 1 : u + 1, pt, q);
            __builtin_amdgcn_sched_barrier(0);
            const float s[3] = {c.s0.x, c.s0.y, c.s0.z}, t[3] = {c.s0.w, c.s1.x, c.s1.y};
            float h1[2], o[2];
            if constexpr (!INV) {
                const float x0 = v[0], x1 = v[1], x2 = v[2];
#pragma unroll
                for (int k = 0; k < 3; ++k)
                    v[k] = fmaf(fc[3 * k + 2], x2, fmaf(fc[3 * k + 1], x1, fmaf(fc[3 * k], x0, fc[9 + k])));
                h1[0] = v[0]; h1[1] = v[1];
                coupling_net<TD>(rec, lane, q, c, h1, o);
                if (TD == 1) { v[1] -= o[0]; v[2] -= o[1]; } else { v[2] -= o[0]; }
                const float y0 = v[2], y1 = v[1], y2 = v[0];
                v[0] = (y0 - t[0]) * expf(-s[0]);
                v[1] = (y1 - t[1]) * expf(-s[1]);
                v[2] = (y2 - t[2]) * expf(-s[2]);
                ld -= (s[0] + s[1]) + s[2];
            } else {
                const float y0 = fmaf(v[0], expf(s[0]), t[0]);
                const float y1 = fmaf(v[1], expf(s[1]), t[1]);
                const float y2 = fmaf(v[2], expf(s[2]), t[2]);
                v[0] = y2; v[1] = y1; v[2] = y0;
                h1[0] = v[0]; h1[1] = v[1];
                coupling_net<TD>(rec, lane, q, c, h1, o);
                if (TD == 1) { v[1] += o[0]; v[2] += o[1]; } else { v[2] += o[0]; }
                const float x0 = v[0], x1 = v[1], x2 = v[2];
#pragma unroll
                for (int k = 0; k < 3; ++k)
                    v[k] = fmaf(fc[12 + 3 * k + 2], x2, fmaf(fc[12 + 3 * k + 1], x1, fmaf(fc[12 + 3 * k], x0, fc[21 + k])));
            }
        });

        if (ok && q == 0) {
            a.out[(size_t)row * 3 + 0] = v[0];
            a.out[(size_t)row * 3 + 1] = v[1];
            a.out[(size_t)row * 3 + 2] = v[2];
            if (!INV) a.ld_pt[row] = ld;
        }
        if constexpr (!INV) {
            if (a.part) {
                float sl = ld;
                float sz = -0.5f * (v[0] * v[0] + LOG2PI_F) + -0.5f * (v[1] * v[1] + LOG2PI_F) + -0.5f * (v[2] * v[2] + LOG2PI_F);
                sl += __shfl_xor(sl, 1); sz += __shfl_xor(sz, 1);
                sl += __shfl_xor(sl, 2); sz += __shfl_xor(sz, 2);
                sl += __shfl_xor(sl, 4); sz += __shfl_xor(sz, 4);
                sl += __shfl_xor(sl, 8); sz += __shfl_xor(sz, 8);
                if (ok && lane == 0) {
                    const int wt = g >> 4;
                    PF_ST(a.part + wt, sl);
                    PF_ST(a.part + (a.rows >> 4) + wt, sz);
                }
            }
        }
    }
    if constexpr (!INV) {
        if (!a.part) return;
        __shared__ float sa[NW * 64];
        __shared__ int is_last;
        asm volatile("s_waitcnt vmcnt(0)" ::: "memory");
        __syncthreads();
        if (threadIdx.x == 0) is_last = atomicAdd(a.counter, 1u) == gridDim.x - 1 ? 1 : 0;
        __syncthreads();
        if (!is_last) return;
        const int tid = threadIdx.x;
        const int per = a.N >> 4, half = a.rows >> 4;
        for (int b = wave; b < a.B; b += NW) {
            float accl = 0.f, accz = 0.f;
            for (int i = lane; i < per; i += 64) {
                accl += PF_LD(a.part + b * per + i);
                accz += PF_LD(a.part + half + b * per + i);
            }
            accl = pf_xor_sum<32, 1>(accl); accz = pf_xor_sum<32, 1>(accz);
            if (lane == 0) {
                const float l = accl + a.ld_const * (float)a.N;
                a.ldj[b] = l;
                a.lps[b] = accz + l;
                if (b < NW * 64) sa[b] = accz + l;
            }
        }
        __syncthreads();
        float tot = 0.f;
        if (tid == 0)
            for (int b = 0; b < a.B; ++b) tot += b < NW * 64 ? sa[b] : a.lps[b];
        if (tid == 0) {
            *a.logp = -tot / (float)a.B;
            PF_ST(a.counter, 0u);
        }
    }
}

template <bool INV, int NW>
int launch_nw(FlowArgs a, hipStream_t s) {
    a.ntiles = (a.rows + NW * 16 - 1) / (NW * 16);
    const int grid = a.ntiles < 256 ? a.ntiles : 256;
    hipLaunchKernelGGL((flow_kernel<INV, NW>), dim3(grid), dim3(NW * 64), 0, s, a);
    return pf_last_launch_status();
}

template <bool INV>
int launch(FlowArgs a, hipStream_t s) {
    constexpr int NWMAX = INV ? PF_FLOW_NW : PF_FLOW_NW_FWD;
    const int wt = (a.rows + 15) / 16;
    if (wt >= 200 * NWMAX) return launch_nw<INV, NWMAX>(a, s);
// ... 95 lines not shown
```

### puflow_amd/csrc/interp.hip

```cpp
#include <hip/hip_runtime.h>
#include "pf_api_internal.h"
#include "pf_mfma.h"
#include "pf_wave.h"

#ifndef PF_INTERP_P
#define PF_INTERP_P 1
#endif
#ifndef PF_INTERP_NW
#define PF_INTERP_NW 12
#endif

namespace {

struct InterpArgs {
    const float* xyz;
    const float* z;
    const int* idx;
    const float* w;
    long long off[15];
    float* u;
    float* aw;
    int T, N, ntiles, R;
    int per;
    int contiguous;
};

template <int P, int NW, bool BIG = false>
__global__ __launch_bounds__(NW * 64) void interp_kernel(InterpArgs a) {
    constexpr int R = 4;
    const int lane = threadIdx.x & 63, wave = threadIdx.x >> 6;
    const int col = lane & 15, q = lane >> 4;
    const int ps = col >> 3, k = col & 7;
    constexpr int L_DT = 0, L_ET = 4, L_WT = 12, L_D3 = 20, L_EC = 28, L_D6 = 44, L_W3 = 60, L_END = 76;
    __shared__ u4 wl[L_END * 128];
    {
        auto stage = [&](int f0, int nf, long long off) {
            const u4* src = reinterpret_cast<const u4*>(a.w + off);
            pf_stage_lds(wl + f0 * 128, src, nf * 128);
        };
        if (a.contiguous) stage(L_DT, L_END, a.off[0]);
        else {
            stage(L_DT, 4, a.off[0]); stage(L_ET, 8, a.off[5]); stage(L_WT, 8, a.off[8]); stage(L_D3, 8, a.off[1]);
            stage(L_EC, 16, a.off[6]); stage(L_D6, 16, a.off[3]); stage(L_W3, 16, a.off[9]);
        }
        __syncthreads();
    }
    const PfW2Lds wsDT{wl + L_DT * 128, lane}, wsET{wl + L_ET * 128, lane}, wsWT{wl + L_WT * 128, lane},
        wsD3{wl + L_D3 * 128, lane}, wsEC{wl + L_EC * 128, lane}, wsD6{wl + L_D6 * 128, lane}, wsW3{wl + L_W3 * 128, lane};
    const PfW2BufD<4> wsW0(a.w + a.off[7], lane);
    const PfW2BufD<2> wsW6(a.w + a.off[BIG ? 13 : 11], lane);

    const float* sc = a.w + a.off[4];
    const float iDT = sc[0], iD3 = sc[1], iW1 = sc[2], iEC = sc[3], iW3 = sc[4], iW6 = sc[5];

    const int wt_end = min((int)(blockIdx.x + 1) * a.per, a.ntiles);
    for (int wt = blockIdx.x * a.per + wave; wt < wt_end; wt += NW) {
        const int pt0 = wt * P * 2;
        int gi[P], gj[P];
        bool ok[P];
        PfPairN e[P][1];
#pragma unroll
        for (int p = 0; p < P; ++p) {
            const int g = pt0 + p * 2 + ps;
            ok[p] = g < a.T;
            gi[p] = ok[p] ? g : a.T - 1;
            gj[p] = (gi[p] / a.N) * a.N + a.idx[(size_t)gi[p] * 16 + k];
            float xi[3], xj[3];
#pragma unroll
            for (int c = 0; c < 3; ++c) {
                xi[c] = a.xyz[(size_t)gi[p] * 3 + c];
                xj[c] = a.xyz[(size_t)gj[p] * 3 + c];
            }
            const float v0 = xi[0] - xj[0], v1 = xi[1] - xj[1], v2 = xi[2] - xj[2];
            const float nrm = sqrtf(__fadd_rn(__fadd_rn(__fmul_rn(v0, v0), __fmul_rn(v1, v1)), __fmul_rn(v2, v2)));
            const f4 z4 = pf_splat(0.f);
            const f4 e0 = {xi[0], xi[1], xi[2], xj[0]}, e1 = {xj[1], xj[2], nrm, 1.f};
            e[p][0] = pf_pairn(q == 0 ? e0 : z4, q == 0 ? e1 : z4);
        }

        f4 w1[P][8];
        {
            PfPairN fp[P][4];
            f4 last[P];
            {
                f4 acc[P][1];
#pragma unroll
                for (int p = 0; p < P; ++p) acc[p][0] = pf_splat(0.f);
                pf_mmn<false, 1, 1, 1>(wsET, 0, e, acc);
#pragma unroll
                for (int p = 0; p < P; ++p) {
                    last[p] = pf_lrelu(acc[p][0] * iEC, 0.05f);
                    fp[p][0] = pf_pairn(last[p], pf_splat(0.f));
                }
            }
            pf_static_for<1, 8>([&](auto tc) {
                constexpr int t = decltype(tc)::value;
                constexpr int CPT = (t + 1) / 2;
                constexpr int F0 = (t / 2) * ((t + 1) / 2);
                f4 acc[P][1];
#pragma unroll
                for (int p = 0; p < P; ++p) acc[p][0] = pf_splat(0.f);
                pf_mmn<false, 1, 1, 1>(wsET, t, e, acc);
                pf_mmn<false, 1, CPT, CPT>(wsEC, F0, fp, acc);
#pragma unroll
                for (int p = 0; p < P; ++p) {
                    const f4 f = pf_lrelu(acc[p][0] * iEC, 0.05f);
                    if constexpr (t % 2 == 1) fp[p][t / 2] = pf_pairn(last[p], f);
                    else fp[p][t / 2] = pf_pairn(f, pf_splat(0.f));
                    last[p] = f;
                }
            });
#pragma unroll
            for (int ob = 0; ob < 8; ++ob)
#pragma unroll
                for (int p = 0; p < P; ++p) w1[p][ob] = pf_splat(0.f);
            pf_mmn<false, 4, 1, 1>(wsWT, 0, e, w1, 0, 0);
            pf_mmn<false, 4, 1, 1>(wsWT, 4, e, w1, 0, 4);
            pf_mmn<false, 4, 4, 4>(wsW0, 0, fp, w1, 0, 0);
            pf_mmn<false, 4, 4, 4>(wsW0, 16, fp, w1, 0, 4);
        }

        {
            f4 d[P][4];
#pragma unroll
            for (int cb = 0; cb < 4; ++cb)
#pragma unroll
                for (int p = 0; p < P; ++p) d[p][cb] = pf_splat(0.f);
            pf_mmn<false, 4, 1, 1>(wsDT, 0, e, d);
            PfPairN dp[P][2];
#pragma unroll
            for (int p = 0; p < P; ++p) {
                dp[p][0] = pf_pairn(pf_lrelu(d[p][0] * iDT, 0.01f), pf_lrelu(d[p][1] * iDT, 0.01f));
                dp[p][1] = pf_pairn(pf_lrelu(d[p][2] * iDT, 0.01f), pf_lrelu(d[p][3] * iDT, 0.01f));
            }
#pragma unroll
            for (int cb = 0; cb < 4; ++cb)
#pragma unroll
                for (int p = 0; p < P; ++p) d[p][cb] = pf_bias(a.w + a.off[2], cb, q);
            pf_mmn<false, 4, 2, 2>(wsD3, 0, dp, d);
#pragma unroll
            for (int p = 0; p < P; ++p) {
                dp[p][0] = pf_pairn(pf_lrelu(d[p][0] * iD3, 0.01f), pf_lrelu(d[p][1] * iD3, 0.01f));
                dp[p][1] = pf_pairn(pf_lrelu(d[p][2] * iD3, 0.01f), pf_lrelu(d[p][3] * iD3, 0.01f));
            }
            pf_mmn<false, 4, 2, 2>(wsD6, 0, dp, w1, 0, 0);
            pf_mmn<false, 4, 2, 2>(wsD6, 8, dp, w1, 0, 4);
        }

        f4 w3[P][BIG ? 2 : 1];
        {
            PfPairN w1p[P][4];
#pragma unroll
            for (int c = 0; c < 4; ++c)
#pragma unroll
                for (int p = 0; p < P; ++p)
                    w1p[p][c] = pf_pairn(pf_lrelu(w1[p][2 * c] * iW1, 0.01f), pf_lrelu(w1[p][2 * c + 1] * iW1, 0.01f));
            f4 w2[P][4];
#pragma unroll
            for (int ob = 0; ob < 4; ++ob)
#pragma unroll
                for (int p = 0; p < P; ++p) w2[p][ob] = pf_bias(a.w + a.off[10], ob, q);
            pf_mmn<false, 4, 4, 4>(wsW3, 0, w1p, w2);
            PfPairN w2p[P][2];
#pragma unroll
            for (int p = 0; p < P; ++p) {
                w2p[p][0] = pf_pairn(pf_lrelu(w2[p][0] * iW3, 0.01f), pf_lrelu(w2[p][1] * iW3, 0.01f));
                w2p[p][1] = pf_pairn(pf_lrelu(w2[p][2] * iW3, 0.01f), pf_lrelu(w2[p][3] * iW3, 0.01f));
            }
#pragma unroll
            for (int p = 0; p < P; ++p)
#pragma unroll
                for (int ob = 0; ob < (BIG ? 2 : 1); ++ob) w3[p][ob] = pf_bias(a.w + a.off[BIG ? 14 : 12], ob, q);
            pf_mmn<false, (BIG ? 2 : 1), 2, 2>(wsW6, 0, w2p, w3);
#pragma unroll
            for (int p = 0; p < P; ++p)
#pragma unroll
                for (int ob = 0; ob < (BIG ? 2 : 1); ++ob) w3[p][ob] = w3[p][ob] * iW6;
        }

#pragma unroll
        for (int p = 0; p < P; ++p) {
            if constexpr (BIG) {
                float zj[3];
#pragma unroll
                for (int c = 0; c < 3; ++c) zj[c] = a.z[(size_t)gj[p] * 3 + c];
#pragma unroll
                for (int ob = 0; ob < 2; ++ob)
#pragma unroll
                    for (int r = 0; r < 4; ++r) {
                        const int row = 16 * ob + 4 * q + r;
                        const float x = w3[p][ob][r];
                        float m = x;
                        m = pf_xor_max<1, 4>(m);
                        const float ex = expf(x - m);
                        float sm = ex;
                        sm = pf_xor_sum<1, 4>(sm);
                        const float av = ex / sm;
#pragma unroll
                        for (int c = 0; c < 3; ++c) {
                            float s = av * zj[c];
                            s = pf_xor_sum<1, 4>(s);
                            if (ok[p] && k == 0 && row < a.R) a.u[((size_t)gi[p] * a.R + row) * 3 + c] = s;
                        }
                    }
            } else {
                float av[R];
#pragma unroll
                for (int r = 0; r < R; ++r) {
                    const float x = w3[p][0][r];
                    float m = x;
                    m = pf_xor_max<1, 4>(m);
                    const float ex = expf(x - m);
                    float s = ex;
                    s = pf_xor_sum<1, 4>(s);
                    av[r] = ex / s;
                }
                if (a.aw) {
                    if (ok[p] && q == 0) {
                        f4 o = {av[0], av[1], av[2], av[3]};
                        *reinterpret_cast<f4*>(a.aw + ((size_t)gi[p] * 8 + k) * 4) = o;
                    }
                    continue;
                }
                const float zj = a.z[(size_t)gj[p] * 3 + (q < 3 ? q : 0)];
#pragma unroll
                for (int r = 0; r < R; ++r) {
                    float s = av[r] * zj;
                    s = pf_xor_sum<1, 4>(s);
                    if (ok[p] && k == 0 && q < 3 && r < a.R) a.u[((size_t)gi[p] * a.R + r) * 3 + q] = s;
                }
            }
        }
    }
}

}

static int interp_launch(const float* xyz, const float* z, const int* idx16, const float* w, const long long* off,
                         float* u_out, float* aw_out, int B, int N, int R, void* stream) {
    if (B <= 0 || N < 8 || (long long)B * N > (1ll << 28)) return PF_ERR_SHAPE;
    if (R < 1 || R > 32) return PF_ERR_UNSUPPORTED;
    constexpr int NWB = 8;
    InterpArgs a{};
    a.xyz = xyz; a.z = z; a.idx = idx16; a.w = w; a.u = u_out; a.aw = aw_out; a.T = B * N; a.N = N; a.R = R;
    for (int i = 0; i < 15; ++i) a.off[i] = off[i];
    a.contiguous = off[5] == off[0] + 4 * 512 && off[8] == off[5] + 8 * 512 && off[1] == off[8] + 8 * 512 &&
                   off[6] == off[1] + 8 * 512 && off[3] == off[6] + 16 * 512 && off[9] == off[3] + 16 * 512;
    auto go = [&](auto pc, auto nwc, auto bigc) {
        constexpr int P = decltype(pc)::value, NW = decltype(nwc)::value;
        constexpr bool BIG = decltype(bigc)::value;
        a.ntiles = (a.T + P * 2 - 1) / (P * 2);
        const int wgt = (a.ntiles + NW - 1) / NW;
        const int grid = wgt < 256 ? wgt : 256;
        a.per = (a.ntiles + grid - 1) / grid;
        hipLaunchKernelGGL((interp_kernel<P, NW, BIG>), dim3(grid), dim3(NW * 64), 0, (hipStream_t)stream, a);
    };
    if (R > 4) go(std::integral_constant<int, 1>{}, std::integral_constant<int, NWB>{}, std::true_type{});
    else go(std::integral_constant<int, PF_INTERP_P>{}, std::integral_constant<int, PF_INTERP_NW>{}, std::false_type{});
    return pf_last_launch_status();
}

extern "C" int pf_interp(const float* xyz, const float* z, const int* idx16, const float* w, const long long* off,
                         float* u_out, int B, int N, int R, void* stream) {
    if (!xyz || !z || !idx16 || !w || !off || !u_out) return PF_ERR_NULL;
    return interp_launch(xyz, z, idx16, w, off, u_out, nullptr, B, N, R, stream);
}

extern "C" int pf_interp_weights(const float* xyz, const int* idx16, const float* w, const long long* off, float* aw_out,
                                 int B, int N, void* stream) {
    if (!xyz || !idx16 || !w || !off || !aw_out) return PF_ERR_NULL;
    return interp_launch(xyz, nullptr, idx16, w, off, nullptr, aw_out, B, N, 4, stream);
}
```

### puflow_amd/csrc/pf_mfma.h

```cpp
#pragma once
#include <hip/hip_runtime.h>
#include <type_traits>
#include "pf_wave.h"

typedef float f4 __attribute__((ext_vector_type(4)));

#define PF_WAVE 64

__device__ __forceinline__ f4 pf_mfma(float a, float b, f4 c) {
    return __builtin_amdgcn_mfma_f32_16x16x4f32(a, b, c, 0, 0, 0);
}

__device__ __forceinline__ f4 pf_splat(float v) { f4 r = {v, v, v, v}; return r; }

__device__ __forceinline__ f4 pf_lrelu(f4 v, float slope) {
    const f4 s = v * slope;
    f4 r;
    r.x = fmaxf(v.x, s.x); r.y = fmaxf(v.y, s.y); r.z = fmaxf(v.z, s.z); r.w = fmaxf(v.w, s.w);
    return r;
}

__device__ __forceinline__ f4 pf_relu(f4 v) {
    f4 r;
    r.x = fmaxf(v.x, 0.f); r.y = fmaxf(v.y, 0.f); r.z = fmaxf(v.z, 0.f); r.w = fmaxf(v.w, 0.f);
// ... 40 lines not shown
                acc[p][acc0 + ob] = pf_mfma(wv[r], in[p][in0 + cb][r], acc[p][acc0 + ob]);
        }
        __builtin_amdgcn_sched_barrier(0);
    }
}

typedef unsigned int u4 __attribute__((ext_vector_type(4)));

typedef _Float16 h8 __attribute__((ext_vector_type(8)));
typedef _Float16 h2 __attribute__((ext_vector_type(2)));
typedef unsigned int u2 __attribute__((ext_vector_type(2)));
constexpr float PF_LO_SCALE = 2048.f, PF_LO_INV = 1.f / 2048.f;

__device__ __forceinline__ u2 pf_split2_pair(float a, float b) {
    unsigned hb = __builtin_bit_cast(unsigned, (h2){(_Float16)a, (_Float16)b});
    asm("" : "+v"(hb));
    const h2 h = __builtin_bit_cast(h2, hb);
    const h2 l = {(_Float16)((a - (float)h.x) * PF_LO_SCALE), (_Float16)((b - (float)h.y) * PF_LO_SCALE)};
    return (u2){hb, __builtin_bit_cast(unsigned, l)};
}

struct PfPair2 { h8 h, l; };
__device__ __forceinline__ PfPair2 pf_pair2(f4 b0, f4 b1) {
    const u2 s0 = pf_split2_pair(b0.x, b0.y), s1 = pf_split2_pair(b0.z, b0.w);
    const u2 s2 = pf_split2_pair(b1.x, b1.y), s3 = pf_split2_pair(b1.z, b1.w);
    PfPair2 p;
    p.h = __builtin_bit_cast(h8, (u4){s0.x, s1.x, s2.x, s3.x});
    p.l = __builtin_bit_cast(h8, (u4){s0.y, s1.y, s2.y, s3.y});
    return p;
}

__device__ __forceinline__ f4 pf_mfma_f16(h8 a, h8 b, f4 c) {
    return __builtin_amdgcn_mfma_f32_16x16x32_f16(a, b, c, 0, 0, 0);
}

#ifndef PF_MM2_DEPTH
#define PF_MM2_DEPTH 8
#endif
#ifndef PF_W2LDS_DEPTH
#define PF_W2LDS_DEPTH 2
#endif
struct PfW2Lds {
    static constexpr int DEPTH = PF_W2LDS_DEPTH;
    const u4* base;
    int lane;
    __device__ __forceinline__ h8 load(int frag, int split) const {
        return __builtin_bit_cast(h8, base[(frag * 2 + split) * PF_WAVE + lane]);
    }
};

template <int DEPTH_>
struct PfW2BufD {
    static constexpr int DEPTH = DEPTH_;
    __amdgpu_buffer_rsrc_t rsrc;
    int voff;
    __device__ __forceinline__ PfW2BufD(const void* p, int lane)
        : rsrc(__builtin_amdgcn_make_buffer_rsrc(const_cast<void*>(p), 0, 0x7fffffff, 0x00020000)), voff(lane * 16) {}
    __device__ __forceinline__ h8 load(int frag, int split) const {
        return __builtin_bit_cast(h8, __builtin_amdgcn_raw_buffer_load_b128(rsrc, voff, (frag * 2 + split) * (PF_WAVE * 16), 0));
    }
};

struct PfW2Buf {
    static constexpr int DEPTH = PF_MM2_DEPTH;
    __amdgpu_buffer_rsrc_t rsrc;
    int voff;
    __device__ __forceinline__ PfW2Buf(const void* p, int lane)
        : rsrc(__builtin_amdgcn_make_buffer_rsrc(const_cast<void*>(p), 0, 0x7fffffff, 0x00020000)), voff(lane * 16) {}
    __device__ __forceinline__ h8 load(int frag, int split) const {
        return __builtin_bit_cast(h8, __builtin_amdgcn_raw_buffer_load_b128(rsrc, voff, (frag * 2 + split) * (PF_WAVE * 16), 0));
    }
};

template <int OB, int CP, int WCP, int D = 2, class WS2, int P, int NIN, int NACC>
__device__ __forceinline__ void pf_mm2(const WS2& ws, int frag0, const PfPair2 (&in)[P][NIN], int in0,
                                       f4 (&acc)[P][NACC], f4 (&accx)[P][NACC], int acc0) {
    constexpr int NFRAG = OB * CP;
    constexpr int DD = D < NFRAG ? D : NFRAG;
    h8 wb[DD][2];
#pragma unroll
    for (int i = 0; i < DD; ++i)
#pragma unroll
        for (int s = 0; s < 2; ++s) wb[i][s] = ws.load(frag0 + (i / CP) * WCP + (i % CP), s);
#pragma unroll
    for (int i = 0; i < NFRAG; ++i) {
        const int ob = i / CP, cp = i % CP;
        const h8 wh = wb[i % DD][0], wl = wb[i % DD][1];
        if (i + DD < NFRAG) {
            const int f = frag0 + ((i + DD) / CP) * WCP + ((i + DD) % CP);
#pragma unroll
            for (int s = 0; s < 2; ++s) wb[i % DD][s] = ws.load(f, s);
        }
#pragma unroll
        for (int p = 0; p < P; ++p) {
            f4 x = accx[p][acc0 + ob];
            x = pf_mfma_f16(wh, in[p][in0 + cp].l, x);
            x = pf_mfma_f16(wl, in[p][in0 + cp].h, x);
            accx[p][acc0 + ob] = x;
            acc[p][acc0 + ob] = pf_mfma_f16(wh, in[p][in0 + cp].h, acc[p][acc0 + ob]);
        }
        __builtin_amdgcn_sched_barrier(0);
    }
}

template <int NB, int P, int NIN>
__device__ __forceinline__ void pf_pairs2(const f4 (&in)[P][NIN], int in0, PfPair2 (&out)[P][(NB + 1) / 2]) {
#pragma unroll
    for (int p = 0; p < P; ++p)
#pragma unroll
        for (int c = 0; c < (NB + 1) / 2; ++c)
            out[p][c] = pf_pair2(in[p][in0 + 2 * c], 2 * c + 1 < NB ? in[p][in0 + 2 * c + 1] : pf_splat(0.f));
}

template <int OB, int CP, int WCP, class WS2, int P, int NIN, int NACC>
__device__ __forceinline__ void pf_mm2f(const WS2& ws, int frag0, const PfPair2 (&in)[P][NIN], int in0,
                                        f4 (&acc)[P][NACC], int acc0) {
    f4 accx[P][OB];
    f4 accm[P][OB];
#pragma unroll
    for (int p = 0; p < P; ++p)
#pragma unroll
        for (int o = 0; o < OB; ++o) { accx[p][o] = pf_splat(0.f); accm[p][o] = acc[p][acc0 + o]; }
    pf_mm2<OB, CP, WCP, WS2::DEPTH>(ws, frag0, in, in0, accm, accx, 0);
#pragma unroll
    for (int p = 0; p < P; ++p)
#pragma unroll
        for (int o = 0; o < OB; ++o) acc[p][acc0 + o] = accm[p][o] + accx[p][o] * PF_LO_INV;
}

struct PfPairN { h8 h, l; };
__device__ __forceinline__ unsigned pf_pk_f16(float a, float b) {
    return __builtin_bit_cast(unsigned, (h2){(_Float16)a, (_Float16)b});
}
__device__ __forceinline__ PfPairN pf_pairn(f4 b0, f4 b1) {
    const unsigned h0 = pf_pk_f16(b0.x, b0.y), h1 = pf_pk_f16(b0.z, b0.w), h2_ = pf_pk_f16(b1.x, b1.y), h3 = pf_pk_f16(b1.z, b1.w);
    unsigned l0, l1, l2, l3;
    asm("v_fma_mixlo_f16 %0, %4, -1.0, %8 op_sel_hi:[1,0,0]\n\t"
        "v_fma_mixlo_f16 %1, %5, -1.0, %10 op_sel_hi:[1,0,0]\n\t"
        "v_fma_mixlo_f16 %2, %6, -1.0, %12 op_sel_hi:[1,0,0]\n\t"
        "v_fma_mixlo_f16 %3, %7, -1.0, %14 op_sel_hi:[1,0,0]\n\t"
        "v_fma_mixhi_f16 %0, %4, -1.0, %9 op_sel:[1,0,0] op_sel_hi:[1,0,0]\n\t"
        "v_fma_mixhi_f16 %1, %5, -1.0, %11 op_sel:[1,0,0] op_sel_hi:[1,0,0]\n\t"
        "v_fma_mixhi_f16 %2, %6, -1.0, %13 op_sel:[1,0,0] op_sel_hi:[1,0,0]\n\t"
        "v_fma_mixhi_f16 %3, %7, -1.0, %15 op_sel:[1,0,0] op_sel_hi:[1,0,0]\n\t"
        "s_nop 1"
        : "=&v"(l0), "=&v"(l1), "=&v"(l2), "=&v"(l3)
        : "v"(h0), "v"(h1), "v"(h2_), "v"(h3), "v"(b0.x), "v"(b0.y), "v"(b0.z), "v"(b0.w), "v"(b1.x), "v"(b1.y), "v"(b1.z), "v"(b1.w));
    PfPairN p;
    p.h = __builtin_bit_cast(h8, (u4){h0, h1, h2_, h3});
    p.l = __builtin_bit_cast(h8, (u4){l0, l1, l2, l3});
    return p;
}

__device__ __forceinline__ float pf_rsmax32(float a, float b) {
    unsigned x = __builtin_bit_cast(unsigned, a), y = __builtin_bit_cast(unsigned, b);
    asm("s_nop 1\n\tv_permlane32_swap_b32 %0, %1" : "+v"(x), "+v"(y));
    return fmaxf(__builtin_bit_cast(float, x), __builtin_bit_cast(float, y));
}
__device__ __forceinline__ float pf_rsmax16(float a, float b) {
    unsigned x = __builtin_bit_cast(unsigned, a), y = __builtin_bit_cast(unsigned, b);
    asm("s_nop 1\n\tv_permlane16_swap_b32 %0, %1" : "+v"(x), "+v"(y));
    return fmaxf(__builtin_bit_cast(float, x), __builtin_bit_cast(float, y));
}

#ifndef PF_MMN_CPMAJOR
#define PF_MMN_CPMAJOR 0
#endif
#ifndef PF_MMN_TERMS
#define PF_MMN_TERMS 3
#endif
#ifndef PF_MMN_PRIO
#define PF_MMN_PRIO 0
#endif
template <bool SWAP, int OB, int CP, int WCP, bool FENCE = true, class WS, int P, int NIN, int NACC>
__device__ __forceinline__ void pf_mmn(const WS& ws, int frag0, const PfPairN (&feat)[P][NIN], f4 (&acc)[P][NACC], int in0 = 0, int acc0 = 0) {
    constexpr int D = WS::DEPTH;
    constexpr int NFRAG = OB * CP;
    constexpr int DD = D < NFRAG ? D : NFRAG;
    auto OBI = [](int i) { return PF_MMN_CPMAJOR ? i % OB : i / CP; };
    auto CPI = [](int i) { return PF_MMN_CPMAJOR ? i / OB : i % CP; };
    h8 wb[DD][2];
#pragma unroll
    for (int i = 0; i < DD; ++i)
#pragma unroll
        for (int s = 0; s < 2; ++s) wb[i][s] = ws.load(frag0 + OBI(i) * WCP + CPI(i), s);
#if PF_MMN_PRIO
    __builtin_amdgcn_s_setprio(PF_MMN_PRIO);
#endif
#pragma unroll
    for (int i = 0; i < NFRAG; ++i) {
        const int ob = OBI(i), cp = CPI(i);
        const h8 wh = wb[i % DD][0], wl = wb[i % DD][1];
        if (i + DD < NFRAG) {
            const int f = frag0 + OBI(i + DD) * WCP + CPI(i + DD);
#pragma unroll
            for (int s = 0; s < 2; ++s) wb[i % DD][s] = ws.load(f, s);
        }
#pragma unroll
        for (int p = 0; p < P; ++p) {
            f4 x = acc[p][acc0 + ob];
            if constexpr (SWAP) {
                if constexpr (PF_MMN_TERMS == 3) {
                    x = pf_mfma_f16(feat[p][in0 + cp].l, wh, x);
                    x = pf_mfma_f16(feat[p][in0 + cp].h, wl, x);
                }
                x = pf_mfma_f16(feat[p][in0 + cp].h, wh, x);
            } else {
                if constexpr (PF_MMN_TERMS == 3) {
                    x = pf_mfma_f16(wh, feat[p][in0 + cp].l, x);
                    x = pf_mfma_f16(wl, feat[p][in0 + cp].h, x);
                }
                x = pf_mfma_f16(wh, feat[p][in0 + cp].h, x);
            }
            acc[p][acc0 + ob] = x;
        }
        if constexpr (FENCE) __builtin_amdgcn_sched_barrier(0);
    }
#if PF_MMN_PRIO
    __builtin_amdgcn_s_setprio(0);
#endif
}


template <int D = 8, class T4>
__device__ __forceinline__ void pf_stage_lds(T4* __restrict__ dst, const T4* __restrict__ src, int n) {
    const int nt = blockDim.x;
    for (int base = threadIdx.x; base < n; base += nt * D) {
        T4 v[D];
#pragma unroll
        for (int k = 0; k < D; ++k) {
            const int i = base + k * nt;
            v[k] = src[i < n ? i : n - 1];
        }
#pragma unroll
        for (int k = 0; k < D; ++k) {
            const int i = base + k * nt;
            if (i < n) dst[i] = v[k];
        }
    }
}

template <int I, int N, class F>
__device__ __forceinline__ void pf_static_for(F&& f) {
    if constexpr (I < N) {
        f(std::integral_constant<int, I>{});
        pf_static_for<I + 1, N>(f);
    }
}

__device__ __forceinline__ f4 pf_bias(const float* __restrict__ b, int ob, int q) {
    return *reinterpret_cast<const f4*>(b + ob * 16 + 4 * q);
}

__device__ __forceinline__ float pf_rowmax16(float v) { return pf_row_reduce(v, PfMax{}); }

__device__ __forceinline__ int pf_xcd_tile(int v, int chunk) { return (v & 7) * chunk + (v >> 3); }
```

### puflow_amd/csrc/pointwise.hip

```cpp
#include <hip/hip_runtime.h>
#include "pf_api_internal.h"
#include "pf_mfma.h"

namespace {

__device__ __forceinline__ h8 pf_ldw(const u4* p) { return __builtin_bit_cast(h8, *p); }

struct PqArgs {
    const float* h;
    const u4* w;
    const float* bias;
    const float* scales;
    float* pq;
    int T, ntiles, NT, nrounds;
    float inv;
};

template <int ODIM, int ROWS, int NW>
__global__ __launch_bounds__(NW * 64) void pq_gemm_kernel(PqArgs a) {
    constexpr int HB = ODIM / 16, CP = (HB + 1) / 2, OBT = ROWS / 16, RB = OBT / NW, NTMAX = 16;
    static_assert(OBT % NW == 0, "rows split evenly over the waves");
    const int lane = threadIdx.x & 63, wave = threadIdx.x >> 6;
    const int col = lane & 15, q = lane >> 4;
    __shared__ u4 bl[NTMAX][CP][2][64];
// ... 5 lines not shown
        for (int cp = 0; cp < CP; ++cp) {
            const u4* f = a.w + (size_t)(((wave * RB + ob) * CP + cp) * 2) * 64 + lane;
            wh[ob][cp] = pf_ldw(f);
            wl[ob][cp] = pf_ldw(f + 64);
        }
        bias[ob] = *reinterpret_cast<const f4*>(a.bias + (wave * RB + ob) * 16 + 4 * q);
    }
    const float inv = a.scales ? a.scales[6] : a.inv;
    for (int round = blockIdx.x; round < a.nrounds; round += gridDim.x) {
        const int tile0 = round * a.NT;
        const int nt = a.ntiles - tile0 < a.NT ? a.ntiles - tile0 : a.NT;
        for (int t = wave; t < nt; t += NW) {
            int pt = (tile0 + t) * 16 + col;
            pt = pt < a.T ? pt : a.T - 1;
            f4 hb[HB + (HB & 1)];
#pragma unroll
            for (int b = 0; b < HB; ++b) hb[b] = *reinterpret_cast<const f4*>(a.h + (size_t)pt * ODIM + b * 16 + 4 * q);
            if constexpr (HB & 1) hb[HB] = pf_splat(0.f);
#pragma unroll
            for (int cp = 0; cp < CP; ++cp) {
                const PfPairN p = pf_pairn(hb[2 * cp], hb[2 * cp + 1]);
                bl[t][cp][0][lane] = __builtin_bit_cast(u4, p.h);
                bl[t][cp][1][lane] = __builtin_bit_cast(u4, p.l);
            }
        }
        __syncthreads();
        for (int t = 0; t < nt; ++t) {
            f4 acc[RB];
#pragma unroll
            for (int ob = 0; ob < RB; ++ob) acc[ob] = pf_splat(0.f);
#pragma unroll
            for (int cp = 0; cp < CP; ++cp) {
                const h8 fh = __builtin_bit_cast(h8, bl[t][cp][0][lane]), fl = __builtin_bit_cast(h8, bl[t][cp][1][lane]);
#pragma unroll
                for (int ob = 0; ob < RB; ++ob) {
                    f4 x = acc[ob];
                    if constexpr (PF_MMN_TERMS == 3) {
                        x = pf_mfma_f16(wh[ob][cp], fl, x);
                        x = pf_mfma_f16(wl[ob][cp], fh, x);
                    }
                    x = pf_mfma_f16(wh[ob][cp], fh, x);
                    acc[ob] = x;
                }
            }
            const int pt = (tile0 + t) * 16 + col;
            if (pt < a.T) {
#pragma unroll
                for (int ob = 0; ob < RB; ++ob) {
                    f4 o;
#pragma unroll
                    for (int r = 0; r < 4; ++r) o[r] = fmaf(acc[ob][r], inv, bias[ob][r]);
                    *reinterpret_cast<f4*>(a.pq + (size_t)pt * ROWS + (wave * RB + ob) * 16 + 4 * q) = o;
                }
            }
        }
        __syncthreads();
    }
}

template <int ODIM, int ROWS>
int launch_pq(PqArgs a, hipStream_t s) {
    constexpr int NW = 16;
    a.ntiles = (a.T + 15) / 16;
    int nt = a.ntiles / 256;
    nt = nt < 1 ? 1 : (nt > 16 ? 16 : nt);
    a.NT = nt;
    a.nrounds = (a.ntiles + nt - 1) / nt;
    const int grid = a.nrounds < 256 ? a.nrounds : 256;
    hipLaunchKernelGGL((pq_gemm_kernel<ODIM, ROWS, NW>), dim3(grid), dim3(NW * 64), 0, s, a);
    return pf_last_launch_status();
}

template <int ODIM>
int launch_ctx(PqArgs a, hipStream_t s) {
    constexpr int NW = 9;
    a.ntiles = (a.T + 15) / 16;
    int nt = a.ntiles / 256;
    nt = nt < 1 ? 1 : (nt > 16 ? 16 : nt);
    a.NT = nt;
    a.nrounds = (a.ntiles + nt - 1) / nt;
    const int grid = a.nrounds < 256 ? a.nrounds : 256;
    hipLaunchKernelGGL((pq_gemm_kernel<ODIM, 288, NW>), dim3(grid), dim3(NW * 64), 0, s, a);
    return pf_last_launch_status();
}

struct CondArgs {
    const float* h;
    const float* w;
    long long off[13];
    float* c;
    float* st;
    float* cp;
    int T, ntiles;
    int contiguous;
};

__device__ __forceinline__ f4 pf_scale(f4 v, float k) { return v * k; }

template <int ODIM>
constexpr int cond_lds_bytes() { return ((ODIM / 32) * ((ODIM / 16 + 1) / 2) + 12 * ((ODIM / 32 + 1) / 2) + 20) * 2048; }

template <int ODIM, int CDIM, int NW>
__device__ __forceinline__ void cond_body(const CondArgs& a, u4* wl, int tile0, int tstride) {
    constexpr int HB = ODIM / 16, MB = ODIM / 32, CB = CDIM / 16;
    constexpr int HP = (HB + 1) / 2, MP = (MB + 1) / 2;
    constexpr int F_M1 = 0, F_H1 = F_M1 + MB * HP, F_S2 = F_H1 + 12 * MP, F_T2 = F_S2 + 8, F_ST4 = F_T2 + 8, F_END = F_ST4 + 4;
    const int lane = threadIdx.x & 63, wave = threadIdx.x >> 6;
    const int col = lane & 15, q = lane >> 4;
    static_assert(F_END * 2048 == cond_lds_bytes<ODIM>(), "LDS size formula");
    {
        auto stage = [&](int f0, int nf, long long off) {
            const u4* src = reinterpret_cast<const u4*>(a.w + off);
            pf_stage_lds(wl + f0 * 128, src, nf * 128);
        };
        if (a.contiguous) stage(F_M1, F_END, a.off[0]);
        else {
            stage(F_M1, MB * HP, a.off[0]); stage(F_H1, 12 * MP, a.off[3]); stage(F_S2, 8, a.off[4]); stage(F_T2, 8, a.off[6]);
            stage(F_ST4, 4, a.off[8]);
        }
        __syncthreads();
    }
    const PfW2Lds wsM1{wl + F_M1 * 128, lane}, wsH1{wl + F_H1 * 128, lane}, wsS2{wl + F_S2 * 128, lane},
        wsT2{wl + F_T2 * 128, lane}, wsST4{wl + F_ST4 * 128, lane};
    const PfW2BufD<2> wsM2(a.w + a.off[2], lane);
    const float* sc = a.w + a.off[12];
    const float iM1 = sc[0], iM2 = sc[1], iH1 = sc[2], iS2 = sc[3], iT2 = sc[4], iST4 = sc[5];
    const float* b1 = a.w + a.off[1];
    const float* bS2 = a.w + a.off[5];
    const float* bT2 = a.w + a.off[7];
    const float* bST4 = a.w + a.off[9];

    const int per = (a.ntiles + tstride - 1) / tstride;
    const int wt_end = min((tile0 + 1) * per, a.ntiles);
    for (int wt = tile0 * per + wave; wt < wt_end; wt += NW) {
        const int g = wt * 16 + col;
        const bool ok = g < a.T;
        const int pt = ok ? g : a.T - 1;
        PfPairN hp[1][HP];
        {
            f4 h[HB + (HB & 1)];
#pragma unroll
            for (int b = 0; b < HB; ++b) h[b] = *reinterpret_cast<const f4*>(a.h + (size_t)pt * ODIM + b * 16 + 4 * q);
            if constexpr (HB & 1) h[HB] = pf_splat(0.f);
#pragma unroll
            for (int c = 0; c < HP; ++c) hp[0][c] = pf_pairn(h[2 * c], h[2 * c + 1]);
        }
        PfPairN mp[1][MP];
        {
            f4 m[1][MB + (MB & 1)];
#pragma unroll
            for (int o = 0; o < MB; ++o) m[0][o] = pf_bias(b1, o, q);
            pf_mmn<false, MB, HP, HP>(wsM1, 0, hp, m);
#pragma unroll
            for (int o = 0; o < MB; ++o) m[0][o] = pf_relu(pf_scale(m[0][o], iM1));
            if constexpr (MB & 1) m[0][MB] = pf_splat(0.f);
#pragma unroll
            for (int c = 0; c < MP; ++c) mp[0][c] = pf_pairn(m[0][2 * c], m[0][2 * c + 1]);
        }
        if (a.c) {
            f4 c[1][CB];
#pragma unroll
            for (int o = 0; o < CB; ++o) c[0][o] = pf_splat(0.f);
            pf_mmn<false, CB, MP, MP>(wsM2, 0, mp, c);
            if (ok)
#pragma unroll
                for (int o = 0; o < CB; ++o)
                    *reinterpret_cast<f4*>(a.c + (size_t)pt * CDIM + o * 16 + 4 * q) = pf_scale(c[0][o], iM2);
        }
        if (!a.st) continue;
        {
            f4 acc[1][4];
#pragma unroll
            for (int o = 0; o < 4; ++o) acc[0][o] = pf_splat(0.f);
            pf_mmn<false, 4, MP, MP>(wsH1, 8 * MP, mp, acc);
            if (ok)
#pragma unroll
                for (int o = 0; o < 4; ++o)
                    *reinterpret_cast<f4*>(a.cp + (size_t)pt * 64 + o * 16 + 4 * q) = pf_scale(acc[0][o], iH1);
        }
        PfPairN h2p[1][4];
        pf_static_for<0, 2>([&](auto nc) {
            constexpr int net = decltype(nc)::value;
            f4 h1[1][4];
#pragma unroll
            for (int o = 0; o < 4; ++o) h1[0][o] = pf_splat(0.f);
            pf_mmn<false, 4, MP, MP>(wsH1, (4 * net) * MP, mp, h1);
            PfPairN h1p[1][2];
            h1p[0][0] = pf_pairn(pf_lrelu(pf_scale(h1[0][0], iH1), 0.01f), pf_lrelu(pf_scale(h1[0][1], iH1), 0.01f));
            h1p[0][1] = pf_pairn(pf_lrelu(pf_scale(h1[0][2], iH1), 0.01f), pf_lrelu(pf_scale(h1[0][3], iH1), 0.01f));
            f4 h2[1][4];
#pragma unroll
            for (int o = 0; o < 4; ++o) h2[0][o] = pf_bias(net == 0 ? bS2 : bT2, o, q);
            if constexpr (net == 0) pf_mmn<false, 4, 2, 2>(wsS2, 0, h1p, h2); else pf_mmn<false, 4, 2, 2>(wsT2, 0, h1p, h2);
            const float i2 = net == 0 ? iS2 : iT2;
            h2p[0][2 * net + 0] = pf_pairn(pf_lrelu(pf_scale(h2[0][0], i2), 0.01f), pf_lrelu(pf_scale(h2[0][1], i2), 0.01f));
            h2p[0][2 * net + 1] = pf_pairn(pf_lrelu(pf_scale(h2[0][2], i2), 0.01f), pf_lrelu(pf_scale(h2[0][3], i2), 0.01f));
        });
        {
            f4 acc[1][1];
            acc[0][0] = pf_bias(bST4, 0, q);
            pf_mmn<false, 1, 4, 4>(wsST4, 0, h2p, acc);
            if (ok && q < 2) *reinterpret_cast<f4*>(a.st + (size_t)pt * 8 + 4 * q) = pf_scale(acc[0][0], iST4);
        }
    }
}

#ifndef PF_COND_NW
#define PF_COND_NW 12
#endif
constexpr int COND_NW = PF_COND_NW;

template <int ODIM, int CDIM>
__global__ __launch_bounds__(COND_NW * 64) void cond_kernel(CondArgs a) {
    extern __shared__ u4 cond_lds[];
    cond_body<ODIM, CDIM, COND_NW>(a, cond_lds, blockIdx.x, gridDim.x);
}

struct CondAllArgs { CondArgs u[6]; int first[7]; };

__global__ __launch_bounds__(COND_NW * 64) void cond_all_kernel(CondAllArgs g) {
    extern __shared__ u4 cond_lds[];
    const int b = blockIdx.x;
    int unit = 0;
#pragma unroll
    for (int i = 1; i < 6; ++i) unit += b >= g.first[i] ? 1 : 0;
    const int slot = b - g.first[unit], n = g.first[unit + 1] - g.first[unit];
    if (unit == 0) cond_body<32, 32, COND_NW>(g.u[0], cond_lds, slot, n);
    else if (unit == 1) cond_body<64, 64, COND_NW>(g.u[1], cond_lds, slot, n);
    else {
        CondArgs a = g.u[2];
        if (unit == 3) a = g.u[3];
        if (unit == 4) a = g.u[4];
        if (unit == 5) a = g.u[5];
        cond_body<128, 128, COND_NW>(a, cond_lds, slot, n);
    }
}

inline int cond_contiguous(const long long* off, int odim) {
    const int HB = odim / 16, MB = odim / 32, HP = (HB + 1) / 2, MP = (MB + 1) / 2;
    long long e = off[0] + (long long)MB * HP * 512;
    if (off[3] != e) return 0;
    e += 12ll * MP * 512;
    if (off[4] != e) return 0;
    e += 8 * 512;
    if (off[6] != e) return 0;
    e += 8 * 512;
    return off[8] == e ? 1 : 0;
}

template <int ODIM, int CDIM>
int launch_cond(CondArgs a, hipStream_t s) {
    constexpr int NW = COND_NW, lds = cond_lds_bytes<ODIM>();
    a.contiguous = cond_contiguous(a.off, ODIM);
    a.ntiles = (a.T + 15) / 16;
    const int wgt = (a.ntiles + NW - 1) / NW;
    int per_cu = (160 * 1024) / lds;
    const int by_waves = 32 / NW;
    if (per_cu > by_waves) per_cu = by_waves;
    if (per_cu < 1) per_cu = 1;
    const int cap = 256 * per_cu;
    const int grid = wgt < cap ? wgt : cap;
    allow_lds(cond_kernel<ODIM, CDIM>, lds);
    hipLaunchKernelGGL((cond_kernel<ODIM, CDIM>), dim3(grid), dim3(NW * 64), lds, s, a);
    return pf_last_launch_status();
}

}

extern "C" int pf_pq_gemm(int unit, const float* h, const float* w, const long long* off, float* pq_next, int T, void* stream) {
    if (!h || !w || !off || !pq_next) return PF_ERR_NULL;
    if (T <= 0) return PF_ERR_SHAPE;
    PqArgs a{};
    a.h = h; a.w = reinterpret_cast<const u4*>(w + off[10]); a.bias = w + off[11]; a.scales = w + off[12]; a.pq = pq_next; a.T = T;
    hipStream_t s = (hipStream_t)stream;
    switch (unit) {
        case 0: return launch_pq<32, 256>(a, s);
        case 1: return launch_pq<64, 512>(a, s);
        case 2: case 3: case 4: return launch_pq<128, 512>(a, s);
        default: return PF_ERR_UNSUPPORTED;
    }
}

extern "C" int pf_cnf_context(const float* c, int cd, const float* hc_image, const float* hb, float inv_scale, float* ctx, int T,
                              void* stream) {
    if (!c || !hc_image || !hb || !ctx) return PF_ERR_NULL;
    if (T <= 0) return PF_ERR_SHAPE;
    PqArgs a{};
    a.h = c; a.w = reinterpret_cast<const u4*>(hc_image); a.bias = hb; a.scales = nullptr; a.inv = inv_scale; a.pq = ctx; a.T = T;
    hipStream_t s = (hipStream_t)stream;
    switch (cd) {
        case 32: return launch_ctx<32>(a, s);
        case 64: return launch_ctx<64>(a, s);
        case 128: return launch_ctx<128>(a, s);
        default: return PF_ERR_UNSUPPORTED;
    }
}

extern "C" int pf_cond(int unit, const float* h, const float* w, const long long* off, float* c, float* st, float* cp,
                       int T, void* stream) {
    if (!h || !w || !off || !st || !cp) return PF_ERR_NULL;
    if (T <= 0) return PF_ERR_SHAPE;
    CondArgs a{};
    a.h = h; a.w = w; a.c = c; a.st = st; a.cp = cp; a.T = T;
    for (int i = 0; i < 13; ++i) a.off[i] = off[i];
    hipStream_t s = (hipStream_t)stream;
    switch (unit) {
        case 0: return launch_cond<32, 32>(a, s);
        case 1: return launch_cond<64, 64>(a, s);
        case 2: case 3: case 4: case 5: return launch_cond<128, 128>(a, s);
        default: return PF_ERR_UNSUPPORTED;
    }
}

extern "C" int pf_cond_all(const float* const* h, const float* w, const long long* off, float* const* c, float* st, float* cp,
                           int T, void* stream) {
    if (!h || !w || !off || (!st != !cp) || (!st && !c)) return PF_ERR_NULL;
    if (T <= 0) return PF_ERR_SHAPE;
    CondAllArgs g{};
    const int ntiles = (T + 15) / 16;
    const int wgt = (ntiles + COND_NW - 1) / COND_NW;
    static const int share_big[6] = {32, 32, 48, 48, 48, 48}, share_small[6] = {24, 32, 50, 50, 50, 50};
    const int* share = wgt <= 50 ? share_small : share_big;
    g.first[0] = 0;
    for (int u = 0; u < 6; ++u) {
        if (!h[u]) return PF_ERR_NULL;
        CondArgs& a = g.u[u];
        a.h = h[u]; a.w = w; a.c = c ? c[u] : nullptr; a.st = st ? st + (size_t)u * T * 8 : nullptr; a.cp = cp ? cp + (size_t)u * T * 64 : nullptr; a.T = T;
        a.ntiles = ntiles;
        for (int i = 0; i < 13; ++i) a.off[i] = off[u * 13 + i];
        a.contiguous = cond_contiguous(a.off, u == 0 ? 32 : (u == 1 ? 64 : 128));
        const int n = wgt < share[u] ? wgt : share[u];
        g.first[u + 1] = g.first[u] + n;
    }
    constexpr int lds = cond_lds_bytes<128>();
    allow_lds(cond_all_kernel, lds);
    hipLaunchKernelGGL(cond_all_kernel, dim3(g.first[6]), dim3(COND_NW * 64), lds, (hipStream_t)stream, g);
    return pf_last_launch_status();
}

extern "C" int pf_post(int unit, const float* h, const float* w, const long long* off, float* c, float* st, float* cp,
                       float* pq_next, int T, void* stream) {
    if (unit < 5) {
        if (!pq_next) return PF_ERR_NULL;
        const int rc = pf_pq_gemm(unit, h, w, off, pq_next, T, stream);
        if (rc != PF_OK) return rc;
    }
    return pf_cond(unit, h, w, off, c, st, cp, T, stream);
}
```

### puflow_amd/packing.py

```python
from __future__ import annotations

from typing import Dict, List

import numpy as np

NUM_BLOCKS = 6
FEAT_CHANNELS = [3, 32, 64, 128, 128, 128, 128]
GROWTH = [8, 16, 32, 32, 32, 32]
COND_CHANNELS = [32, 64, 128, 128, 128, 128]
HDIM = 64
BN_EPS = 1e-5


def _np(sd, k):
    return sd[k].detach().cpu().numpy().astype(np.float64)


def _fold_bn(sd, conv: str, bn: str):
    W = _np(sd, conv + ".weight")
    W = W.reshape(W.shape[0], -1)
    b = _np(sd, conv + ".bias")
    s = _np(sd, bn + ".weight") / np.sqrt(_np(sd, bn + ".running_var") + BN_EPS)
    return W * s[:, None], s * (b - _np(sd, bn + ".running_mean")) + _np(sd, bn + ".bias")

# ... 140 lines not shown

def frag_pack_f16n(W: np.ndarray) -> np.ndarray:
    out, inn = W.shape
    OB, CP = (out + 15) // 16, (inn + 31) // 32
    Wp = np.zeros((OB * 16, CP * 32), dtype=np.float32)
    Wp[:out, :inn] = W
    if np.abs(Wp).max(initial=0.0) >= 65504.0:
        raise ValueError("scaled weight magnitude exceeds the fp16 range of the f16n path; use ec_mode='f32'")
    hi = Wp.astype(np.float16)
    lo = (Wp - hi.astype(np.float32)).astype(np.float32).astype(np.float16)
    lanes = np.arange(64)
    row, q = lanes & 15, lanes >> 4
    j = np.arange(8)
    ch = np.where(j[None, :] < 4, 4 * q[:, None] + j[None, :], 16 + 4 * q[:, None] + (j[None, :] - 4))
    res = np.zeros((OB, CP, 2, 64, 8), dtype=np.uint16)
    for si, part in enumerate((hi, lo)):
        bits = part.view(np.uint16).reshape(OB, 16, CP, 32)
        res[:, :, si] = bits.reshape(OB, 16, CP, 2, 4, 4).transpose(0, 2, 4, 1, 3, 5).reshape(OB, CP, 64, 8)
    return res.reshape(-1).view(np.float32)


def f16n_scale(W: np.ndarray) -> float:
    m = float(np.abs(W).max(initial=0.0))
    if m == 0.0 or not np.isfinite(m):
        return 1.0
    return float(2.0 ** int(np.clip(13 - np.floor(np.log2(m)), -24, 40)))


def frag_pack_f16n_scaled(W: np.ndarray):
    sc = f16n_scale(W)
    return frag_pack_f16n((W.astype(np.float64) * sc).astype(np.float32)), np.float32(1.0 / sc)


EC4_STEP = 4.0


def ec4_scales(nconv: int = 4, g: int = 32, odim: int = 128):
    a = EC4_STEP ** np.arange(nconv + 1)
    S = g * nconv + odim
    rp = np.ones(S); rq = np.ones(S)
    for t in range(nconv):
        rp[g * t:g * (t + 1)] = a[t]; rq[g * t:g * (t + 1)] = a[t]
    rq[g * nconv:] = a[nconv]
    return rp.astype(np.float32), rq.astype(np.float32), a.astype(np.float32)


def ec4_weights(u: Dict[str, np.ndarray], nconv: int = 4, g: int = 32) -> np.ndarray:
    _, _, a = ec4_scales(nconv, g, u[f"G{nconv}"].shape[0])
    parts = []
    for t in range(1, nconv + 1):
        Gt = u[f"G{t}"].astype(np.float64).copy()
        for c in range(t):
            Gt[:, g * c:g * (c + 1)] *= a[t] / a[c]
        parts.append(frag_pack_f16n(Gt.astype(np.float32)))
    return np.concatenate(parts)


def frag_unpack_f16x2(F: np.ndarray, out: int, inn: int) -> np.ndarray:
    OB, CP = (out + 15) // 16, (inn + 31) // 32
    img = np.ascontiguousarray(F, dtype=np.float32).view(np.uint16).reshape(OB, CP, 2, 64, 8).view(np.float16).astype(np.float64)
    val = img[:, :, 0] + img[:, :, 1] / F16_LO_SCALE
    lanes = np.arange(64)
    row, q = lanes & 15, lanes >> 4
    j = np.arange(8)
    ch = np.where(j[None, :] < 4, 4 * q[:, None] + j[None, :], 16 + 4 * q[:, None] + (j[None, :] - 4))
    W = np.zeros((OB, 16, CP, 32))
    W[:, row[:, None], :, ch] = val.transpose(2, 3, 0, 1)
    return W.reshape(OB * 16, CP * 32)[:out, :inn]


def frag_unpack_f16n(F: np.ndarray, out: int, inn: int) -> np.ndarray:
    OB, CP = (out + 15) // 16, (inn + 31) // 32
    img = np.ascontiguousarray(F, dtype=np.float32).view(np.uint16).reshape(OB, CP, 2, 64, 8).view(np.float16).astype(np.float64)
    val = img[:, :, 0] + img[:, :, 1]
    lanes = np.arange(64)
    row, q = lanes & 15, lanes >> 4
    j = np.arange(8)
    ch = np.where(j[None, :] < 4, 4 * q[:, None] + j[None, :], 16 + 4 * q[:, None] + (j[None, :] - 4))
    W = np.zeros((OB, 16, CP, 32))
    W[:, row[:, None], :, ch] = val.transpose(2, 3, 0, 1)
    return W.reshape(OB * 16, CP * 32)[:out, :inn]


def frag_unpack(F: np.ndarray, out: int, inn: int) -> np.ndarray:
    OB, CB = F.shape[0], F.shape[1]
    f = F.reshape(OB, CB, 4, 16, 4).transpose(0, 3, 1, 2, 4)
    return f.reshape(OB * 16, CB * 16)[:out, :inn]


POST_SLOTS = ["M1", "b1", "M2", "H1", "S2", "bS2", "T2", "bT2", "ST4", "bST4", "PQ", "bPQ", "scales"]
POST_SCALES = ["M1", "M2", "H1", "S2", "T2", "ST4", "PQ"]
INTERP_SLOTS = ["dtab", "d_W3", "d_b3", "d_W6", "scales", "ectab", "ec_w", "w_W0", "w_b0", "w_W3", "w_b3", "w_W6", "w_b6",
                "w_W6full", "w_b6full"]
INTERP_SCALES = ["dtab", "d_W3", "w1", "ec", "w_W3", "w_W6"]
FLOW_REC = 5360


class _Blob:
    def __init__(self):
        self.parts: List[np.ndarray] = []
        self.n = 0

    def add(self, a: np.ndarray) -> int:
        a = np.ascontiguousarray(a, dtype=np.float32).reshape(-1)
        off = self.n
        pad = (-a.size) % 64
        self.parts.append(a)
        if pad:
            self.parts.append(np.zeros(pad, np.float32))
        self.n += a.size + pad
        return off

    def data(self) -> np.ndarray:
        return np.concatenate(self.parts) if self.parts else np.zeros(0, np.float32)


def _pad_vec(v: np.ndarray, n: int) -> np.ndarray:
    out = np.zeros(n, np.float32)
    out[:v.size] = v
    return out


def _edge_table(u: Dict[str, np.ndarray]) -> np.ndarray:
    S = u["PA"].shape[0]
    t = np.zeros((S, 8), np.float32)
    t[:, 0:3], t[:, 3:6], t[:, 6] = u["PA"], u["QB"], u["pb"]
    return t


def _etab_dense(xi: np.ndarray, xj: np.ndarray, nrm, const: np.ndarray) -> np.ndarray:
    rows = xi.shape[0]
    W = np.zeros((rows, 32), np.float32)
    W[:, 0:3] = xi
    W[:, 3] = xj[:, 0]
    W[:, 16:18] = xj[:, 1:3]
    if nrm is not None:
        W[:, 18] = nrm
    W[:, 19] = const
    return W


def _etab_frag(xi: np.ndarray, xj: np.ndarray, nrm, const: np.ndarray) -> np.ndarray:
    rows = xi.shape[0]
    W = np.zeros((rows, 32), np.float32)
    W[:, 0:3] = xi
    W[:, 3] = xj[:, 0]
    W[:, 16:18] = xj[:, 1:3]
    if nrm is not None:
        W[:, 18] = nrm
    W[:, 19] = const
    return frag_pack_f16x2(W)


def _ec_frags(u: Dict[str, np.ndarray], nconv: int) -> np.ndarray:
    return np.concatenate([frag_pack(u[f"G{t}"]).reshape(-1) for t in range(1, nconv + 1)])


def pack_flow_record(f: Dict[str, object]) -> np.ndarray:
    rec = np.zeros(FLOW_REC, np.float32)
    img2, inv2 = frag_pack_f16n_scaled(f["c1_W2"])
    rec[0:4096] = img2
    W4 = f["c1_W4"]
    W4r = np.zeros((16, 64), np.float32)
    b4r = np.zeros(16, np.float32)
    for q in range(4):
        W4r[4 * q:4 * q + W4.shape[0]] = W4
        b4r[4 * q:4 * q + W4.shape[0]] = f["c1_b4"]
    img4, inv4 = frag_pack_f16n_scaled(W4r)
    rec[4096:5120] = img4
    rec[5120:5184] = f["c1_b2"] / inv2
    rec[5184:5200] = b4r / inv4
    W0h = np.zeros((64, 2), np.float32)
    W0h[:, :f["tdim"]] = f["c1_W0h"]
    rec[5200:5328] = W0h.reshape(-1)
    rec[5328:5337] = f["A"].reshape(-1); rec[5337:5340] = f["a0"]
    rec[5340:5349] = f["Ai"].reshape(-1); rec[5349:5352] = f["ai0"]
    rec[5352], rec[5353] = inv2, inv4
    return rec


def pack_plan(plan: Dict[str, object], ec_mode: str = "f16n") -> Dict[str, object]:
    if ec_mode not in ("f16n", "f32"):
        raise ValueError(f"unknown EdgeConv arithmetic mode {ec_mode!r}")
    B = _Blob()
    out: Dict[str, object] = {}
    units = plan["units"]
    out["ec_tab0"] = B.add(_edge_table(units[0]))
    out["ec_w"] = [B.add(_ec_frags(units[i], 4)) for i in range(NUM_BLOCKS)]
    out["ec4_w"] = [None, None] + [B.add(ec4_weights(units[i])) for i in range(2, NUM_BLOCKS)]
    ec1n = []
    for i in range(2):
        parts = [ec4_weights(units[i], 4, 16)]
        if i == 0:
            rp, rq, _ = ec4_scales(4, 16, 32)
            parts.append(frag_pack_f16n(_etab_dense(units[0]["PA"] * rq[:, None], units[0]["QB"] * rq[:, None], None, units[0]["pb"] * rq)))
        ec1n.append(B.add(np.concatenate(parts)))
    out["ec1n_w"] = ec1n + [None] * (NUM_BLOCKS - 2)
    out["ec_mode"] = ec_mode
    post = []
    for i in range(NUM_BLOCKS):
        m, f = plan["merges"][i], plan["flows"][i]
        H1 = (np.concatenate([f["s_W0"], f["t_W0"], f["c1_W0c"]], axis=0).astype(np.float64)
              @ m["W2"].astype(np.float64)).astype(np.float32)
        ST4 = np.zeros((6, 128), np.float32)
        ST4[0:3, 0:64] = f["s_W4"]; ST4[3:6, 64:128] = f["t_W4"]
        bST4 = _pad_vec(np.concatenate([f["s_b4"], f["t_b4"]]), 16)
        inv = {}
        def img(name, W):
            im, inv[name] = frag_pack_f16n_scaled(W)
            return B.add(im)
        offs = {"M1": img("M1", m["W1"]), "H1": img("H1", H1), "S2": img("S2", f["s_W2"]), "T2": img("T2", f["t_W2"]),
                "ST4": img("ST4", ST4)}
        assert offs["ST4"] + 4 * 512 == B.n and (B.n - offs["M1"]) % 512 == 0
        offs["M2"] = img("M2", m["W2"])
        offs["b1"] = B.add(_pad_vec(m["b1"], ((m["b1"].size + 15) // 16) * 16) / inv["M1"])
        offs["bS2"] = B.add(f["s_b2"] / inv["S2"]); offs["bT2"] = B.add(f["t_b2"] / inv["T2"])
        offs["bST4"] = B.add(bST4 / inv["ST4"])
        if i + 1 < NUM_BLOCKS:
            nu = units[i + 1]
            Wpq = np.concatenate([nu["PA"], nu["QB"]], axis=0)
            bpq = np.concatenate([nu["pb"], np.zeros_like(nu["pb"])])
            if ec_mode == "f16n":
                rp, rq, _ = ec4_scales() if i + 1 >= 2 else ec4_scales(4, 16, 64)
                rs = np.concatenate([rp, rq])
                Wpq, bpq = Wpq * rs[:, None], bpq * rs
            offs["PQ"] = img("PQ", Wpq)
            offs["bPQ"] = B.add(bpq)
        else:
            offs["PQ"], offs["bPQ"], inv["PQ"] = 0, 0, np.float32(1.0)
        offs["scales"] = B.add(_pad_vec(np.array([inv[k] for k in POST_SCALES], np.float32), 16))
        post.append([offs[k] for k in POST_SLOTS])
    out["post"] = post
    out["flow"] = B.add(np.concatenate([pack_flow_record(f) for f in plan["flows"]]))
    out["ld_const"] = float(sum(f["ld_const"] for f in plan["flows"]))
    ip = plan["interp"]
    W6r = np.zeros((16, 64), np.float32)
    b6r = np.zeros(16, np.float32)
    for q in range(4):
        W6r[4 * q:4 * q + 4] = ip["w_W6"][:4]
        b6r[4 * q:4 * q + 4] = ip["w_b6"][:4]
    ec = ip["ec"]
    ft = ip["f_tab"]
    def grp(*mats):
        sc = min(f16n_scale(m) for m in mats)
        return sc, [frag_pack_f16n((m.astype(np.float64) * sc).astype(np.float32)) for m in mats]
    dtab_d = _etab_dense(ip["d_PA"], ip["d_QB"], ip["d_wn"], ip["d_b0"])
    ectab_d = _etab_dense(ec["PA"][:128], ec["QB"][:128], None, ec["pb"][:128])
    w1tab_d = _etab_dense(ft[:, 0:3], ft[:, 3:6], None, ft[:, 6] + ip["f_b0"])
    s_dt, (i_dt,) = grp(dtab_d)
    s_d3, (i_d3,) = grp(ip["d_W3"])
    s_w1, (i_w1t, i_d6, i_w0) = grp(w1tab_d, ip["f_dW"], ip["f_eW"])
    ecG = [ec[f"G{t}"] for t in range(1, 8)]
    s_ec, ec_imgs = grp(ectab_d, *ecG)
    s_w3, (i_w3,) = grp(ip["w_W3"])
    s_w6, (i_w6r, i_w6f) = grp(W6r, ip["w_W6"])
    io = {}
    for k, im in (("dtab", i_dt), ("ectab", ec_imgs[0]), ("w_b0", i_w1t), ("d_W3", i_d3), ("ec_w", np.concatenate(ec_imgs[1:])),
                  ("d_W6", i_d6), ("w_W3", i_w3)):
        io[k] = B.add(im)
    assert B.n - io["dtab"] == 76 * 512
    io.update({
        "d_b3": B.add(ip["d_b3"] * s_d3),
        "scales": B.add(_pad_vec(np.array([1 / s_dt, 1 / s_d3, 1 / s_w1, 1 / s_ec, 1 / s_w3, 1 / s_w6], np.float32), 16)),
        "w_W0": B.add(i_w0),
        "w_b3": B.add(ip["w_b3"] * s_w3),
        "w_W6": B.add(i_w6r), "w_b6": B.add(b6r * s_w6),
        "w_W6full": B.add(i_w6f), "w_b6full": B.add(ip["w_b6"] * s_w6),
    })
    out["interp"] = [io[k] for k in INTERP_SLOTS]
    out["blob"] = B.data()
    return out


CNF_REC = 10160
CNF_CTX = 288


def _np32(t) -> np.ndarray:
    return t.detach().cpu().numpy().astype(np.float32) if hasattr(t, "detach") else np.asarray(t, np.float32)


LOG2E = 1.4426950408889634


def pack_cnf_context(Hc: np.ndarray):
    return frag_pack_f16n_scaled(np.ascontiguousarray(Hc, dtype=np.float32))


def cnf_split_ok(rec, T_end: float) -> bool:
    tv = np.asarray(rec[9872:9872 + CNF_CTX], np.float64)
    g = np.concatenate([tv[0:64], tv[128:192], tv[256:272]])
    return bool(np.abs(g).max() * abs(T_end) <= 100.0)


CNF_GRAD = 4900
CNF_GRAD_TV = 4612
CNF_CTX_SLOTS = ((0, 64), (64, 64), (128, 64), (192, 64), (256, 3), (272, 3))


def cnf_hyper_matrix(sd, i: int) -> np.ndarray:
    p = f"flow_blocks.{i}.cnf.odefunc.diffeq.layers"
    first = _np32(sd[f"{p}.0._hyper_gate.weight"])
    H = np.zeros((CNF_CTX, first.shape[1]), np.float32)
    for l in range(3):
        for kind, base in (("_hyper_gate", 128 * l), ("_hyper_bias", 128 * l + (64 if l < 2 else 16))):
            W = _np32(sd[f"{p}.{l}.{kind}.weight"])
            for r0 in ([base] if l < 2 else [base + 4 * qq for qq in range(4)]):
                H[r0:r0 + W.shape[0]] = W
    return H


def unpack_cnf_grads(i: int, grad, dH, dhb):
    import torch
    p = f"flow_blocks.{i}.cnf.odefunc.diffeq.layers"
    out = {
        f"{p}.1._layer.weight": grad[0:4096].reshape(64, 64), f"{p}.0._layer.weight": grad[4096:4288].reshape(64, 3),
        f"{p}.0._layer.bias": grad[4288:4352], f"{p}.1._layer.bias": grad[4352:4416],
        f"{p}.2._layer.weight": grad[4416:4608].reshape(3, 64), f"{p}.2._layer.bias": grad[4608:4611],
    }
    tv = grad[CNF_GRAD_TV:CNF_GRAD]
    for l in range(3):
        (g0, n), (b0, _) = CNF_CTX_SLOTS[2 * l], CNF_CTX_SLOTS[2 * l + 1]
        out[f"{p}.{l}._hyper_gate.weight"] = torch.cat([tv[g0:g0 + n, None], dH[g0:g0 + n]], dim=1)
        out[f"{p}.{l}._hyper_gate.bias"] = dhb[g0:g0 + n]
        out[f"{p}.{l}._hyper_bias.weight"] = torch.cat([tv[b0:b0 + n, None], dH[b0:b0 + n]], dim=1)
    return {k: v.contiguous() for k, v in out.items()}


def pack_cnf_block(sd, i: int):
    p = f"flow_blocks.{i}.cnf.odefunc.diffeq.layers"
    L = [{k: _np32(sd[f"{p}.{j}.{k}"]) for k in ("_layer.weight", "_layer.bias", "_hyper_bias.weight",
                                               "_hyper_gate.weight", "_hyper_gate.bias")} for j in range(3)]
    cdim = L[0]["_hyper_gate.weight"].shape[1] - 1
    Hc = np.zeros((CNF_CTX, cdim), np.float32)
    hb = np.zeros(CNF_CTX, np.float32)
    tv = np.zeros(CNF_CTX, np.float32)

    def put(row0, Wg, bg, rep):
        rows = Wg.shape[0]
        for qq in range(4 if rep else 1):
            r0 = row0 + 4 * qq if rep else row0
            Hc[r0:r0 + rows] = Wg[:, 1:]
            tv[r0:r0 + rows] = Wg[:, 0]
            if bg is not None:
                hb[r0:r0 + rows] = bg

    put(0, L[0]["_hyper_gate.weight"], L[0]["_hyper_gate.bias"], False)
    put(64, L[0]["_hyper_bias.weight"], None, False)
    put(128, L[1]["_hyper_gate.weight"], L[1]["_hyper_gate.bias"], False)
    put(192, L[1]["_hyper_bias.weight"], None, False)
    put(256, L[2]["_hyper_gate.weight"], L[2]["_hyper_gate.bias"], True)
    put(272, L[2]["_hyper_bias.weight"], None, True)
    for lo, hi, f in ((0, 64, -LOG2E), (128, 192, -LOG2E), (256, 272, -LOG2E), (64, 128, 2 * LOG2E), (192, 256, 2 * LOG2E)):
        Hc[lo:hi] *= np.float32(f); hb[lo:hi] *= np.float32(f); tv[lo:hi] *= np.float32(f)

    rec = np.zeros(CNF_REC, np.float32)
    W1, W2, W3 = L[0]["_layer.weight"], L[1]["_layer.weight"], L[2]["_layer.weight"]
    rec[0:4096] = frag_pack_f16x2((W2.astype(np.float64) * (2 * LOG2E)).astype(np.float32))
    rec[4096:8192] = frag_pack_f16x2(np.ascontiguousarray(W2.T))
    W3r = np.zeros((16, 64), np.float32)
    b3r = np.zeros(16, np.float32)
    for qq in range(4):
        W3r[4 * qq:4 * qq + 3] = W3
        b3r[4 * qq:4 * qq + 3] = L[2]["_layer.bias"]
    rec[8192:9216] = frag_pack_f16x2(W3r)
    W1t = np.zeros((64, 4), np.float32); W1t[:, :3] = W1; W1t[:, 3] = L[0]["_layer.bias"]
    W1t = (W1t.astype(np.float64) * (2 * LOG2E)).astype(np.float32)
    W3t = np.zeros((64, 4), np.float32); W3t[:, :3] = W3.T
    rec[9216:9472] = W1t.reshape(-1)
    rec[9472:9728] = W3t.reshape(-1)
    rec[9728:9792] = L[0]["_layer.bias"]
    rec[9792:9856] = (L[1]["_layer.bias"].astype(np.float64) * (2 * LOG2E)).astype(np.float32)
    rec[9856:9872] = b3r
    rec[9872:10160] = tv
    T_end = float(_np32(sd[f"flow_blocks.{i}.cnf.sqrt_end_time"])) ** 2
    return rec, Hc, hb, T_end
```

Measured before the change: 27110 patches/s.

## Use single-MFMA edge tables and fused split-fp16 activation packing

```diff
diff --git a/include/puflow_hip.h b/include/puflow_hip.h
--- a/include/puflow_hip.h
+++ b/include/puflow_hip.h
@@ -33,6 +33,8 @@
             void* stream);
 int pf_post(int unit, const float* h, const float* w, const long long* off, float* c, float* st, float* cp,
             float* pq_next, int T, void* stream);
+int pf_test_act_pairn(const float* x, int n, float inv, float slope, unsigned* old_h, unsigned* old_l, unsigned* new_h,
+                      unsigned* new_l, void* stream);
 int pf_cond_all(const float* const* h, const float* w, const long long* off, float* const* c, float* st, float* cp, int T,
                 void* stream);
 
diff --git a/puflow_amd/_lib.py b/puflow_amd/_lib.py
--- a/puflow_amd/_lib.py
+++ b/puflow_amd/_lib.py
@@ -73,6 +73,7 @@
     "pf_post": (c_int, [c_int, c_void_p, c_void_p, POINTER(c_longlong), c_void_p, c_void_p, c_void_p, c_void_p, c_int,
                         c_void_p]),
     "pf_pq_gemm": (c_int, [c_int, c_void_p, c_void_p, POINTER(c_longlong), c_void_p, c_int, c_void_p]),
+    "pf_test_act_pairn": (c_int, [c_void_p, c_int, c_float, c_float, c_void_p, c_void_p, c_void_p, c_void_p, c_void_p]),
     "pf_cond_all": (c_int, [POINTER(c_void_p), c_void_p, POINTER(c_longlong), POINTER(c_void_p), c_void_p, c_void_p, c_int, c_void_p]),
     "pf_cond": (c_int, [c_int, c_void_p, c_void_p, POINTER(c_longlong), c_void_p, c_void_p, c_void_p, c_int, c_void_p]),
     "pf_flow_fwd": (c_int, [c_void_p, c_void_p, c_void_p, c_void_p, c_void_p, c_void_p, c_int, c_void_p]),
diff --git a/puflow_amd/build.py b/puflow_amd/build.py
--- a/puflow_amd/build.py
+++ b/puflow_amd/build.py
@@ -11,6 +11,10 @@
 FLAGS = ["--offload-arch=gfx950", "-O3", "-std=c++17", "-fPIC", "-ffp-contract=on", "-Wno-unused-result"]
 EXTRA_FLAGS = {s: ["-fno-honor-nans", "-mllvm", "-amdgpu-mfma-vgpr-form=" + os.environ.get("PF_MFMA_VGPR_FORM", "1")] for s in ("edgeconv.hip", "pointwise.hip", "flow.hip", "interp.hip", "cnf.hip", "cnf_bwd.hip")}
 EXTRA_FLAGS["edgeconv.hip"] = EXTRA_FLAGS["edgeconv.hip"] + ["-DPF_W2LDS_DEPTH=" + os.environ.get("PF_EC_W2LDS_DEPTH", "3")]
+_PACKED = os.environ.get("PF_PACKED_FP32", "").split(",")
+for _s in ("edgeconv.hip", "pointwise.hip", "flow.hip", "interp.hip"):
+    if _s not in _PACKED:
+        EXTRA_FLAGS[_s] = EXTRA_FLAGS[_s] + ["-Xclang", "-target-feature", "-Xclang", "-packed-fp32-ops"]
 if os.environ.get("PF_INTERP_TRACKERS", "1") != "0":
     EXTRA_FLAGS["interp.hip"] = EXTRA_FLAGS["interp.hip"] + ["-mllvm", "-amdgpu-use-amdgpu-trackers=1"]
 
diff --git a/puflow_amd/csrc/edgeconv.hip b/puflow_amd/csrc/edgeconv.hip
--- a/puflow_amd/csrc/edgeconv.hip
+++ b/puflow_amd/csrc/edgeconv.hip
@@ -1,6 +1,12 @@
 #include <hip/hip_runtime.h>
 #include "pf_api_internal.h"
 #include "pf_mfma.h"
+
+#if defined(__HIP_DEVICE_COMPILE__)
+#define PF_PACKED_FP32_FN __attribute__((target("packed-fp32-ops")))
+#else
+#define PF_PACKED_FP32_FN
+#endif
 
 namespace {
 
@@ -237,7 +243,7 @@
 constexpr float EC4_OUT_INV = 1.f / 256.f;
 
 template <int P, int NW, int DBG = 0, bool PQF = false>
-__global__ __launch_bounds__(NW * 64) void edgeconv4_kernel(EcArgs a) {
+__global__ __launch_bounds__(NW * 64) PF_PACKED_FP32_FN void edgeconv4_kernel(EcArgs a) {
     static_assert(!PQF || NW * P == 16, "the fused P|Q GEMM takes a workgroup tile of 16 points as one MFMA column tile");
     constexpr int NCONV = 4, G = 32, S = 256, OBO = 8, OCH = 2, ODIM = 128;
     constexpr int NWF = 2 * (NCONV * (NCONV - 1) / 2) + OBO * NCONV;
@@ -404,7 +410,8 @@
     static_assert(!PQF || NW * P == 16, "the fused P|Q GEMM takes a workgroup tile of 16 points as one MFMA column tile");
     constexpr int NCONV = 4, S = 16 * NCONV + ODIM, SB = S / 16, OBO = ODIM / 16;
     constexpr int PQ_ROWS = ODIM == 32 ? 256 : 512;
-    constexpr int FO = 4, FT = FO + OBO * 2, NWF = FT + (C3 ? SB : 0);
+    constexpr int FO = 4, FT = FO + OBO * 2, NWF = FT + (C3 ? SB / 2 : 0);
+    static_assert(!C3 || SB % 2 == 0, "the edge table fills whole 2-KiB slots");
     constexpr int ROWB = 2 * S * 4;
     static_assert(OBO == 2 || OBO == 4, "reduce-scatter below is written for 2 or 4 output blocks");
     const int lane = threadIdx.x & 63, wave = threadIdx.x >> 6;
@@ -416,6 +423,7 @@
     pf_stage_lds(wlds, reinterpret_cast<const u4*>(a.wg), NWF * 128);
     __syncthreads();
     const PfW2Lds ws{wlds, lane};
+    const float inv_tab = C3 ? reinterpret_cast<const float*>(a.wg)[NWF * 512] : 1.f;
     const __amdgpu_buffer_rsrc_t rs = __builtin_amdgcn_make_buffer_rsrc(const_cast<float*>(C3 ? a.xyz : a.pq), 0, 0x7fffffff, 0x00020000);
 
     for (int v = blockIdx.x; v < 8 * a.chunk; v += gridDim.x) {
@@ -423,7 +431,7 @@
         if (tile >= a.ntiles) continue;
         const int pt0 = (tile * NW + wave) * P;
         int gi[P], vQ[P], vO[P][4];
-        PfPairN e[P][1];
+        h8 e[P];
 #pragma unroll
         for (int p = 0; p < P; ++p) {
             int g = pt0 + p;
@@ -439,9 +447,8 @@
                     xi[c] = a.xyz[(size_t)g * 3 + c];
                     xj[c] = a.xyz[(size_t)jc * 3 + c];
                 }
-                const f4 z4 = pf_splat(0.f);
                 const f4 e0 = {xi[0], xi[1], xi[2], xj[0]}, e1 = {xj[1], xj[2], 0.f, 1.f};
-                e[p][0] = pf_pairn(q == 0 ? e0 : z4, q == 0 ? e1 : z4);
+                e[p] = pf_edge_operand(e0, e1, q);
             } else {
                 const int4 j4 = *reinterpret_cast<const int4*>(a.idx + (size_t)g * 16 + 4 * q);
                 vQ[p] = jc * ROWB + (S + 4 * q) * 4;
@@ -466,8 +473,16 @@
 #pragma unroll
                 for (int b = 0; b < OBO; ++b) outi[p][b] = pf_splat(0.f);
             }
-            pf_mmn<false, NCONV, 1, 1>(ws, FT, e, pre);
-            pf_mmn<true, OBO, 1, 1>(ws, FT + NCONV, e, outi);
+            const PfW1Lds wt{wlds + FT * 128, lane};
+            pf_mm1<false, NCONV>(wt, 0, e, pre);
+            pf_mm1<true, OBO>(wt, NCONV, e, outi);
+#pragma unroll
+            for (int p = 0; p < P; ++p) {
+#pragma unroll
+                for (int b = 0; b < NCONV; ++b) pre[p][b] = pre[p][b] * inv_tab;
+#pragma unroll
+                for (int b = 0; b < OBO; ++b) outi[p][b] = outi[p][b] * inv_tab;
+            }
         } else {
 #pragma unroll
             for (int b = 0; b < NCONV; ++b)
@@ -488,11 +503,11 @@
         }
 
         PfPairN fp[P][2];
-        f4 last[P];
+        PfHalfN last[P];
 #pragma unroll
         for (int p = 0; p < P; ++p) {
-            last[p] = pf_lrelu(pre[p][0], 0.05f);
-            fp[p][0] = pf_pairn(last[p], pf_splat(0.f));
+            last[p] = pf_act_halfn(pre[p][0], 0.05f);
+            fp[p][0] = pf_join_halfn(last[p], PfHalfN{});
         }
         pf_static_for<1, NCONV>([&](auto tc) {
             constexpr int t = decltype(tc)::value;
@@ -503,9 +518,9 @@
             pf_mmn<false, 1, CPT, CPT>(ws, F0, fp, acc);
 #pragma unroll
             for (int p = 0; p < P; ++p) {
-                const f4 f = pf_lrelu(acc[p][0], 0.05f);
-                if constexpr (t % 2 == 1) fp[p][t / 2] = pf_pairn(last[p], f);
-                else fp[p][t / 2] = pf_pairn(f, pf_splat(0.f));
+                const PfHalfN f = pf_act_halfn(acc[p][0], 0.05f);
+                if constexpr (t % 2 == 1) fp[p][t / 2] = pf_join_halfn(last[p], f);
+                else fp[p][t / 2] = pf_join_halfn(f, PfHalfN{});
                 last[p] = f;
             }
         });
diff --git a/puflow_amd/csrc/flow.hip b/puflow_amd/csrc/flow.hip
--- a/puflow_amd/csrc/flow.hip
+++ b/puflow_amd/csrc/flow.hip
@@ -68,18 +68,18 @@
                 v.x = fmaf(wa.y, h1[1], v.x); v.y = fmaf(wa.w, h1[1], v.y);
                 v.z = fmaf(wb.y, h1[1], v.z); v.w = fmaf(wb.w, h1[1], v.w);
             }
-            hid[cb] = pf_lrelu(v, 0.01f);
-        }
-        hp[0][0] = pf_pairn(hid[0], hid[1]);
-        hp[0][1] = pf_pairn(hid[2], hid[3]);
+            hid[cb] = v;
+        }
+        hp[0][0] = pf_act_pairn(hid[0], hid[1], 0.01f);
+        hp[0][1] = pf_act_pairn(hid[2], hid[3], 0.01f);
     }
     const PfW2Lds ws{reinterpret_cast<const u4*>(rec), lane};
     f4 h2[1][4];
 #pragma unroll
     for (int ob = 0; ob < 4; ++ob) h2[0][ob] = pf_bias(rec + 5120, ob, q);
     pf_mmn<false, 4, 2, 2>(ws, 0, hp, h2);
-    hp[0][0] = pf_pairn(pf_lrelu(h2[0][0] * i2, 0.01f), pf_lrelu(h2[0][1] * i2, 0.01f));
-    hp[0][1] = pf_pairn(pf_lrelu(h2[0][2] * i2, 0.01f), pf_lrelu(h2[0][3] * i2, 0.01f));
+    hp[0][0] = pf_act_pairn(h2[0][0], h2[0][1], i2, 0.01f);
+    hp[0][1] = pf_act_pairn(h2[0][2], h2[0][3], i2, 0.01f);
     f4 acc[1][1];
     acc[0][0] = *reinterpret_cast<const f4*>(rec + 5184 + 4 * q);
     pf_mmn<false, 1, 2, 2>(ws, 8, hp, acc);
diff --git a/puflow_amd/csrc/interp.hip b/puflow_amd/csrc/interp.hip
--- a/puflow_amd/csrc/interp.hip
+++ b/puflow_amd/csrc/interp.hip
@@ -31,7 +31,7 @@
     const int lane = threadIdx.x & 63, wave = threadIdx.x >> 6;
     const int col = lane & 15, q = lane >> 4;
     const int ps = col >> 3, k = col & 7;
-    constexpr int L_DT = 0, L_ET = 4, L_WT = 12, L_D3 = 20, L_EC = 28, L_D6 = 44, L_W3 = 60, L_END = 76;
+    constexpr int L_DT = 0, L_ET = 2, L_WT = 6, L_D3 = 10, L_EC = 18, L_D6 = 34, L_W3 = 50, L_END = 66;
     __shared__ u4 wl[L_END * 128];
     {
         auto stage = [&](int f0, int nf, long long off) {
@@ -40,13 +40,13 @@
         };
         if (a.contiguous) stage(L_DT, L_END, a.off[0]);
         else {
-            stage(L_DT, 4, a.off[0]); stage(L_ET, 8, a.off[5]); stage(L_WT, 8, a.off[8]); stage(L_D3, 8, a.off[1]);
+            stage(L_DT, 2, a.off[0]); stage(L_ET, 4, a.off[5]); stage(L_WT, 4, a.off[8]); stage(L_D3, 8, a.off[1]);
             stage(L_EC, 16, a.off[6]); stage(L_D6, 16, a.off[3]); stage(L_W3, 16, a.off[9]);
         }
         __syncthreads();
     }
-    const PfW2Lds wsDT{wl + L_DT * 128, lane}, wsET{wl + L_ET * 128, lane}, wsWT{wl + L_WT * 128, lane},
-        wsD3{wl + L_D3 * 128, lane}, wsEC{wl + L_EC * 128, lane}, wsD6{wl + L_D6 * 128, lane}, wsW3{wl + L_W3 * 128, lane};
+    const PfW1Lds wsDT{wl + L_DT * 128, lane}, wsET{wl + L_ET * 128, lane}, wsWT{wl + L_WT * 128, lane};
+    const PfW2Lds wsD3{wl + L_D3 * 128, lane}, wsEC{wl + L_EC * 128, lane}, wsD6{wl + L_D6 * 128, lane}, wsW3{wl + L_W3 * 128, lane};
     const PfW2BufD<4> wsW0(a.w + a.off[7], lane);
     const PfW2BufD<2> wsW6(a.w + a.off[BIG ? 13 : 11], lane);
 
@@ -58,7 +58,7 @@
         const int pt0 = wt * P * 2;
         int gi[P], gj[P];
         bool ok[P];
-        PfPairN e[P][1];
+        h8 e[P];
 #pragma unroll
         for (int p = 0; p < P; ++p) {
             const int g = pt0 + p * 2 + ps;
@@ -73,24 +73,23 @@
             }
             const float v0 = xi[0] - xj[0], v1 = xi[1] - xj[1], v2 = xi[2] - xj[2];
             const float nrm = sqrtf(__fadd_rn(__fadd_rn(__fmul_rn(v0, v0), __fmul_rn(v1, v1)), __fmul_rn(v2, v2)));
-            const f4 z4 = pf_splat(0.f);
             const f4 e0 = {xi[0], xi[1], xi[2], xj[0]}, e1 = {xj[1], xj[2], nrm, 1.f};
-            e[p][0] = pf_pairn(q == 0 ? e0 : z4, q == 0 ? e1 : z4);
+            e[p] = pf_edge_operand(e0, e1, q);
         }
 
         f4 w1[P][8];
         {
             PfPairN fp[P][4];
-            f4 last[P];
+            PfHalfN last[P];
             {
                 f4 acc[P][1];
 #pragma unroll
                 for (int p = 0; p < P; ++p) acc[p][0] = pf_splat(0.f);
-                pf_mmn<false, 1, 1, 1>(wsET, 0, e, acc);
+                pf_mm1<false, 1>(wsET, 0, e, acc);
 #pragma unroll
                 for (int p = 0; p < P; ++p) {
-                    last[p] = pf_lrelu(acc[p][0] * iEC, 0.05f);
-                    fp[p][0] = pf_pairn(last[p], pf_splat(0.f));
+                    last[p] = pf_act_halfn(acc[p][0], iEC, 0.05f);
+                    fp[p][0] = pf_join_halfn(last[p], PfHalfN{});
                 }
             }
             pf_static_for<1, 8>([&](auto tc) {
@@ -100,13 +99,13 @@
                 f4 acc[P][1];
 #pragma unroll
                 for (int p = 0; p < P; ++p) acc[p][0] = pf_splat(0.f);
-                pf_mmn<false, 1, 1, 1>(wsET, t, e, acc);
+                pf_mm1<false, 1>(wsET, t, e, acc);
                 pf_mmn<false, 1, CPT, CPT>(wsEC, F0, fp, acc);
 #pragma unroll
                 for (int p = 0; p < P; ++p) {
-                    const f4 f = pf_lrelu(acc[p][0] * iEC, 0.05f);
-                    if constexpr (t % 2 == 1) fp[p][t / 2] = pf_pairn(last[p], f);
-                    else fp[p][t / 2] = pf_pairn(f, pf_splat(0.f));
+                    const PfHalfN f = pf_act_halfn(acc[p][0], iEC, 0.05f);
+                    if constexpr (t % 2 == 1) fp[p][t / 2] = pf_join_halfn(last[p], f);
+                    else fp[p][t / 2] = pf_join_halfn(f, PfHalfN{});
                     last[p] = f;
                 }
             });
@@ -114,8 +113,8 @@
             for (int ob = 0; ob < 8; ++ob)
 #pragma unroll
                 for (int p = 0; p < P; ++p) w1[p][ob] = pf_splat(0.f);
-            pf_mmn<false, 4, 1, 1>(wsWT, 0, e, w1, 0, 0);
-            pf_mmn<false, 4, 1, 1>(wsWT, 4, e, w1, 0, 4);
+            pf_mm1<false, 4>(wsWT, 0, e, w1, 0);
+            pf_mm1<false, 4>(wsWT, 4, e, w1, 4);
             pf_mmn<false, 4, 4, 4>(wsW0, 0, fp, w1, 0, 0);
             pf_mmn<false, 4, 4, 4>(wsW0, 16, fp, w1, 0, 4);
         }
@@ -126,12 +125,12 @@
             for (int cb = 0; cb < 4; ++cb)
 #pragma unroll
                 for (int p = 0; p < P; ++p) d[p][cb] = pf_splat(0.f);
-            pf_mmn<false, 4, 1, 1>(wsDT, 0, e, d);
+            pf_mm1<false, 4>(wsDT, 0, e, d);
             PfPairN dp[P][2];
 #pragma unroll
             for (int p = 0; p < P; ++p) {
-                dp[p][0] = pf_pairn(pf_lrelu(d[p][0] * iDT, 0.01f), pf_lrelu(d[p][1] * iDT, 0.01f));
-                dp[p][1] = pf_pairn(pf_lrelu(d[p][2] * iDT, 0.01f), pf_lrelu(d[p][3] * iDT, 0.01f));
+                dp[p][0] = pf_act_pairn(d[p][0], d[p][1], iDT, 0.01f);
+                dp[p][1] = pf_act_pairn(d[p][2], d[p][3], iDT, 0.01f);
             }
 #pragma unroll
             for (int cb = 0; cb < 4; ++cb)
@@ -140,8 +139,8 @@
             pf_mmn<false, 4, 2, 2>(wsD3, 0, dp, d);
 #pragma unroll
             for (int p = 0; p < P; ++p) {
-                dp[p][0] = pf_pairn(pf_lrelu(d[p][0] * iD3, 0.01f), pf_lrelu(d[p][1] * iD3, 0.01f));
-                dp[p][1] = pf_pairn(pf_lrelu(d[p][2] * iD3, 0.01f), pf_lrelu(d[p][3] * iD3, 0.01f));
+                dp[p][0] = pf_act_pairn(d[p][0], d[p][1], iD3, 0.01f);
+                dp[p][1] = pf_act_pairn(d[p][2], d[p][3], iD3, 0.01f);
             }
             pf_mmn<false, 4, 2, 2>(wsD6, 0, dp, w1, 0, 0);
             pf_mmn<false, 4, 2, 2>(wsD6, 8, dp, w1, 0, 4);
@@ -154,7 +153,7 @@
             for (int c = 0; c < 4; ++c)
 #pragma unroll
                 for (int p = 0; p < P; ++p)
-                    w1p[p][c] = pf_pairn(pf_lrelu(w1[p][2 * c] * iW1, 0.01f), pf_lrelu(w1[p][2 * c + 1] * iW1, 0.01f));
+                    w1p[p][c] = pf_act_pairn(w1[p][2 * c], w1[p][2 * c + 1], iW1, 0.01f);
             f4 w2[P][4];
 #pragma unroll
             for (int ob = 0; ob < 4; ++ob)
@@ -164,8 +163,8 @@
             PfPairN w2p[P][2];
 #pragma unroll
             for (int p = 0; p < P; ++p) {
-                w2p[p][0] = pf_pairn(pf_lrelu(w2[p][0] * iW3, 0.01f), pf_lrelu(w2[p][1] * iW3, 0.01f));
-                w2p[p][1] = pf_pairn(pf_lrelu(w2[p][2] * iW3, 0.01f), pf_lrelu(w2[p][3] * iW3, 0.01f));
+                w2p[p][0] = pf_act_pairn(w2[p][0], w2[p][1], iW3, 0.01f);
+                w2p[p][1] = pf_act_pairn(w2[p][2], w2[p][3], iW3, 0.01f);
             }
 #pragma unroll
             for (int p = 0; p < P; ++p)
@@ -244,7 +243,7 @@
     InterpArgs a{};
     a.xyz = xyz; a.z = z; a.idx = idx16; a.w = w; a.u = u_out; a.aw = aw_out; a.T = B * N; a.N = N; a.R = R;
     for (int i = 0; i < 15; ++i) a.off[i] = off[i];
-    a.contiguous = off[5] == off[0] + 4 * 512 && off[8] == off[5] + 8 * 512 && off[1] == off[8] + 8 * 512 &&
+    a.contiguous = off[5] == off[0] + 4 * 256 && off[8] == off[5] + 8 * 256 && off[1] == off[8] + 8 * 256 &&
                    off[6] == off[1] + 8 * 512 && off[3] == off[6] + 16 * 512 && off[9] == off[3] + 16 * 512;
     auto go = [&](auto pc, auto nwc, auto bigc) {
         constexpr int P = decltype(pc)::value, NW = decltype(nwc)::value;
diff --git a/puflow_amd/csrc/pf_mfma.h b/puflow_amd/csrc/pf_mfma.h
--- a/puflow_amd/csrc/pf_mfma.h
+++ b/puflow_amd/csrc/pf_mfma.h
@@ -216,6 +216,74 @@
     return p;
 }
 
+__device__ __forceinline__ float pf_opaque(float v) { asm("" : "+v"(v)); return v; }
+
+enum { PF_ACT_LRELU = 0, PF_ACT_RELU = 1 };
+template <bool SCALE, int ACT>
+__device__ __forceinline__ float pf_act1n(float v, float inv, float slope) {
+    if constexpr (SCALE) v = v * inv;
+    if constexpr (ACT == PF_ACT_RELU) return pf_opaque(fmaxf(v, 0.f));
+    else return pf_opaque(fmaxf(v, v * slope));
+}
+
+struct PfHalfN { u2 h, l; };
+__device__ __forceinline__ PfHalfN pf_splitn4(float x0, float x1, float x2, float x3) {
+    const unsigned h0 = pf_pk_f16(x0, x1), h1 = pf_pk_f16(x2, x3);
+    unsigned l0, l1;
+    asm("v_fma_mixlo_f16 %0, %2, -1.0, %4 op_sel_hi:[1,0,0]\n\t"
+        "v_fma_mixlo_f16 %1, %3, -1.0, %6 op_sel_hi:[1,0,0]\n\t"
+        "v_fma_mixhi_f16 %0, %2, -1.0, %5 op_sel:[1,0,0] op_sel_hi:[1,0,0]\n\t"
+        "v_fma_mixhi_f16 %1, %3, -1.0, %7 op_sel:[1,0,0] op_sel_hi:[1,0,0]\n\t"
+        "s_nop 1"
+        : "=&v"(l0), "=&v"(l1)
+        : "v"(h0), "v"(h1), "v"(x0), "v"(x1), "v"(x2), "v"(x3));
+    return PfHalfN{(u2){h0, h1}, (u2){l0, l1}};
+}
+__device__ __forceinline__ PfPairN pf_splitn8(float x0, float x1, float x2, float x3, float x4, float x5, float x6, float x7) {
+    const unsigned h0 = pf_pk_f16(x0, x1), h1 = pf_pk_f16(x2, x3), h2_ = pf_pk_f16(x4, x5), h3 = pf_pk_f16(x6, x7);
+    unsigned l0, l1, l2, l3;
+    asm("v_fma_mixlo_f16 %0, %4, -1.0, %8 op_sel_hi:[1,0,0]\n\t"
+        "v_fma_mixlo_f16 %1, %5, -1.0, %10 op_sel_hi:[1,0,0]\n\t"
+        "v_fma_mixlo_f16 %2, %6, -1.0, %12 op_sel_hi:[1,0,0]\n\t"
+        "v_fma_mixlo_f16 %3, %7, -1.0, %14 op_sel_hi:[1,0,0]\n\t"
+        "v_fma_mixhi_f16 %0, %4, -1.0, %9 op_sel:[1,0,0] op_sel_hi:[1,0,0]\n\t"
+        "v_fma_mixhi_f16 %1, %5, -1.0, %11 op_sel:[1,0,0] op_sel_hi:[1,0,0]\n\t"
+        "v_fma_mixhi_f16 %2, %6, -1.0, %13 op_sel:[1,0,0] op_sel_hi:[1,0,0]\n\t"
+        "v_fma_mixhi_f16 %3, %7, -1.0, %15 op_sel:[1,0,0] op_sel_hi:[1,0,0]\n\t"
+        "s_nop 1"
+        : "=&v"(l0), "=&v"(l1), "=&v"(l2), "=&v"(l3)
+        : "v"(h0), "v"(h1), "v"(h2_), "v"(h3), "v"(x0), "v"(x1), "v"(x2), "v"(x3), "v"(x4), "v"(x5), "v"(x6), "v"(x7));
+    PfPairN p;
+    p.h = __builtin_bit_cast(h8, (u4){h0, h1, h2_, h3});
+    p.l = __builtin_bit_cast(h8, (u4){l0, l1, l2, l3});
+    return p;
+}
+
+template <bool SCALE, int ACT>
+__device__ __forceinline__ PfPairN pf_act_pairn_t(f4 b0, f4 b1, float inv, float slope) {
+    return pf_splitn8(pf_act1n<SCALE, ACT>(b0.x, inv, slope), pf_act1n<SCALE, ACT>(b0.y, inv, slope),
+                      pf_act1n<SCALE, ACT>(b0.z, inv, slope), pf_act1n<SCALE, ACT>(b0.w, inv, slope),
+                      pf_act1n<SCALE, ACT>(b1.x, inv, slope), pf_act1n<SCALE, ACT>(b1.y, inv, slope),
+                      pf_act1n<SCALE, ACT>(b1.z, inv, slope), pf_act1n<SCALE, ACT>(b1.w, inv, slope));
+}
+template <bool SCALE, int ACT>
+__device__ __forceinline__ PfHalfN pf_act_halfn_t(f4 b, float inv, float slope) {
+    return pf_splitn4(pf_act1n<SCALE, ACT>(b.x, inv, slope), pf_act1n<SCALE, ACT>(b.y, inv, slope),
+                      pf_act1n<SCALE, ACT>(b.z, inv, slope), pf_act1n<SCALE, ACT>(b.w, inv, slope));
+}
+__device__ __forceinline__ PfPairN pf_act_pairn(f4 b0, f4 b1, float inv, float slope) { return pf_act_pairn_t<true, PF_ACT_LRELU>(b0, b1, inv, slope); }
+__device__ __forceinline__ PfPairN pf_act_pairn(f4 b0, f4 b1, float slope) { return pf_act_pairn_t<false, PF_ACT_LRELU>(b0, b1, 1.f, slope); }
+__device__ __forceinline__ PfPairN pf_relu_pairn(f4 b0, f4 b1, float inv) { return pf_act_pairn_t<true, PF_ACT_RELU>(b0, b1, inv, 0.f); }
+__device__ __forceinline__ PfHalfN pf_act_halfn(f4 b, float inv, float slope) { return pf_act_halfn_t<true, PF_ACT_LRELU>(b, inv, slope); }
+__device__ __forceinline__ PfHalfN pf_act_halfn(f4 b, float slope) { return pf_act_halfn_t<false, PF_ACT_LRELU>(b, 1.f, slope); }
+__device__ __forceinline__ PfHalfN pf_relu_halfn(f4 b, float inv) { return pf_act_halfn_t<true, PF_ACT_RELU>(b, inv, 0.f); }
+__device__ __forceinline__ PfPairN pf_join_halfn(PfHalfN a, PfHalfN b) {
+    PfPairN p;
+    p.h = __builtin_bit_cast(h8, (u4){a.h.x, a.h.y, b.h.x, b.h.y});
+    p.l = __builtin_bit_cast(h8, (u4){a.l.x, a.l.y, b.l.x, b.l.y});
+    return p;
+}
+
 __device__ __forceinline__ float pf_rsmax32(float a, float b) {
     unsigned x = __builtin_bit_cast(unsigned, a), y = __builtin_bit_cast(unsigned, b);
     asm("s_nop 1\n\tv_permlane32_swap_b32 %0, %1" : "+v"(x), "+v"(y));
@@ -285,6 +353,32 @@
 #endif
 }
 
+struct PfW1Lds {
+    const u4* base;
+    int lane;
+    __device__ __forceinline__ h8 load(int frag) const { return __builtin_bit_cast(h8, base[frag * PF_WAVE + lane]); }
+};
+__device__ __forceinline__ h8 pf_edge_operand(f4 e0, f4 e1, int q) {
+    const PfPairN s = pf_pairn(e0, e1);
+    const u4 h = __builtin_bit_cast(u4, s.h), l = __builtin_bit_cast(u4, s.l), z = {0u, 0u, 0u, 0u};
+    if constexpr (PF_MMN_TERMS == 3) return __builtin_bit_cast(h8, q == 1 ? l : (q == 3 ? z : h));
+    else return __builtin_bit_cast(h8, q == 0 ? h : z);
+}
+template <bool SWAP, int OB, class WS, int P, int NACC>
+__device__ __forceinline__ void pf_mm1(const WS& ws, int frag0, const h8 (&e)[P], f4 (&acc)[P][NACC], int acc0 = 0) {
+    h8 w[OB];
+#pragma unroll
+    for (int ob = 0; ob < OB; ++ob) w[ob] = ws.load(frag0 + ob);
+#pragma unroll
+    for (int ob = 0; ob < OB; ++ob) {
+#pragma unroll
+        for (int p = 0; p < P; ++p) {
+            if constexpr (SWAP) acc[p][acc0 + ob] = pf_mfma_f16(e[p], w[ob], acc[p][acc0 + ob]);
+            else acc[p][acc0 + ob] = pf_mfma_f16(w[ob], e[p], acc[p][acc0 + ob]);
+        }
+    }
+    __builtin_amdgcn_sched_barrier(0);
+}
 
 template <int D = 8, class T4>
 __device__ __forceinline__ void pf_stage_lds(T4* __restrict__ dst, const T4* __restrict__ src, int n) {
diff --git a/puflow_amd/csrc/pointwise.hip b/puflow_amd/csrc/pointwise.hip
--- a/puflow_amd/csrc/pointwise.hip
+++ b/puflow_amd/csrc/pointwise.hip
@@ -181,10 +181,10 @@
             for (int o = 0; o < MB; ++o) m[0][o] = pf_bias(b1, o, q);
             pf_mmn<false, MB, HP, HP>(wsM1, 0, hp, m);
 #pragma unroll
-            for (int o = 0; o < MB; ++o) m[0][o] = pf_relu(pf_scale(m[0][o], iM1));
-            if constexpr (MB & 1) m[0][MB] = pf_splat(0.f);
-#pragma unroll
-            for (int c = 0; c < MP; ++c) mp[0][c] = pf_pairn(m[0][2 * c], m[0][2 * c + 1]);
+            for (int c = 0; c < MP; ++c) {
+                if (2 * c + 1 < MB) mp[0][c] = pf_relu_pairn(m[0][2 * c], m[0][2 * c + 1], iM1);
+                else mp[0][c] = pf_join_halfn(pf_relu_halfn(m[0][2 * c], iM1), PfHalfN{});
+            }
         }
         if (a.c) {
             f4 c[1][CB];
@@ -215,15 +215,15 @@
             for (int o = 0; o < 4; ++o) h1[0][o] = pf_splat(0.f);
             pf_mmn<false, 4, MP, MP>(wsH1, (4 * net) * MP, mp, h1);
             PfPairN h1p[1][2];
-            h1p[0][0] = pf_pairn(pf_lrelu(pf_scale(h1[0][0], iH1), 0.01f), pf_lrelu(pf_scale(h1[0][1], iH1), 0.01f));
-            h1p[0][1] = pf_pairn(pf_lrelu(pf_scale(h1[0][2], iH1), 0.01f), pf_lrelu(pf_scale(h1[0][3], iH1), 0.01f));
+            h1p[0][0] = pf_act_pairn(h1[0][0], h1[0][1], iH1, 0.01f);
+            h1p[0][1] = pf_act_pairn(h1[0][2], h1[0][3], iH1, 0.01f);
             f4 h2[1][4];
 #pragma unroll
             for (int o = 0; o < 4; ++o) h2[0][o] = pf_bias(net == 0 ? bS2 : bT2, o, q);
             if constexpr (net == 0) pf_mmn<false, 4, 2, 2>(wsS2, 0, h1p, h2); else pf_mmn<false, 4, 2, 2>(wsT2, 0, h1p, h2);
             const float i2 = net == 0 ? iS2 : iT2;
-            h2p[0][2 * net + 0] = pf_pairn(pf_lrelu(pf_scale(h2[0][0], i2), 0.01f), pf_lrelu(pf_scale(h2[0][1], i2), 0.01f));
-            h2p[0][2 * net + 1] = pf_pairn(pf_lrelu(pf_scale(h2[0][2], i2), 0.01f), pf_lrelu(pf_scale(h2[0][3], i2), 0.01f));
+            h2p[0][2 * net + 0] = pf_act_pairn(h2[0][0], h2[0][1], i2, 0.01f);
+            h2p[0][2 * net + 1] = pf_act_pairn(h2[0][2], h2[0][3], i2, 0.01f);
         });
         {
             f4 acc[1][1];
@@ -376,3 +376,27 @@
     }
     return pf_cond(unit, h, w, off, c, st, cp, T, stream);
 }
+
+namespace {
+__global__ void act_pairn_test_kernel(const float* __restrict__ x, int n8, float inv, float slope, u4* __restrict__ old_h,
+                                      u4* __restrict__ old_l, u4* __restrict__ new_h, u4* __restrict__ new_l) {
+    const int i = blockIdx.x * blockDim.x + threadIdx.x;
+    if (i >= n8) return;
+    const f4 b0 = *reinterpret_cast<const f4*>(x + (size_t)i * 8), b1 = *reinterpret_cast<const f4*>(x + (size_t)i * 8 + 4);
+    const PfPairN o = pf_pairn(pf_lrelu(pf_scale(b0, inv), slope), pf_lrelu(pf_scale(b1, inv), slope));
+    const PfPairN n = inv == 1.f ? pf_act_pairn(b0, b1, slope) : pf_act_pairn(b0, b1, inv, slope);
+    old_h[i] = __builtin_bit_cast(u4, o.h); old_l[i] = __builtin_bit_cast(u4, o.l);
+    new_h[i] = __builtin_bit_cast(u4, n.h); new_l[i] = __builtin_bit_cast(u4, n.l);
+}
+}
+
+extern "C" int pf_test_act_pairn(const float* x, int n, float inv, float slope, unsigned* old_h, unsigned* old_l,
+                                 unsigned* new_h, unsigned* new_l, void* stream) {
+    if (!x || !old_h || !old_l || !new_h || !new_l) return PF_ERR_NULL;
+    if (n <= 0 || n % 8 != 0) return PF_ERR_SHAPE;
+    const int n8 = n / 8;
+    hipLaunchKernelGGL(act_pairn_test_kernel, dim3((n8 + 63) / 64), dim3(64), 0, (hipStream_t)stream, x, n8, inv, slope,
+                       reinterpret_cast<u4*>(old_h), reinterpret_cast<u4*>(old_l), reinterpret_cast<u4*>(new_h),
+                       reinterpret_cast<u4*>(new_l));
+    return pf_last_launch_status();
+}
diff --git a/puflow_amd/packing.py b/puflow_amd/packing.py
--- a/puflow_amd/packing.py
+++ b/puflow_amd/packing.py
@@ -316,6 +316,42 @@
     return frag_pack_f16x2(W)
 
 
+_ETAB_COLS = np.array([0, 1, 2, 3, 16, 17, 18, 19])
+
+
+def _etab_frag1(W: np.ndarray) -> np.ndarray:
+    rows = W.shape[0]
+    OB = (rows + 15) // 16
+    Wp = np.zeros((OB * 16, 32), dtype=np.float32)
+    Wp[:rows] = W
+    rest = np.ones(32, bool); rest[_ETAB_COLS] = False
+    if np.any(Wp[:, rest] != 0):
+        raise ValueError("not an edge table: columns outside 0..3 / 16..19 are in use")
+    if np.abs(Wp).max(initial=0.0) >= 65504.0:
+        raise ValueError("scaled weight magnitude exceeds the fp16 range of the f16n path; use ec_mode='f32'")
+    hi = Wp.astype(np.float16)
+    lo = (Wp - hi.astype(np.float32)).astype(np.float32).astype(np.float16)
+    D = np.zeros((OB * 16, 32), dtype=np.float16)
+    D[:, _ETAB_COLS] = hi[:, _ETAB_COLS]
+    D[:, _ETAB_COLS + 4] = hi[:, _ETAB_COLS]
+    D[:, _ETAB_COLS + 8] = lo[:, _ETAB_COLS]
+    res = D.view(np.uint16).reshape(OB, 16, 2, 4, 4).transpose(0, 3, 1, 2, 4).reshape(OB, 64, 8)
+    return np.ascontiguousarray(res).reshape(-1).view(np.float32)
+
+
+def etab_unpack_frag1(F: np.ndarray, rows: int):
+    OB = (rows + 15) // 16
+    img = np.ascontiguousarray(F, dtype=np.float32).view(np.uint16).reshape(OB, 4, 16, 8).view(np.float16).astype(np.float64)
+    return tuple(img[:, q].reshape(OB * 16, 8)[:rows] for q in range(4))
+
+
+def ec1n_unit0_table(u: Dict[str, np.ndarray]):
+    _, rq, _ = ec4_scales(4, 16, 32)
+    T = _etab_dense(u["PA"] * rq[:, None], u["QB"] * rq[:, None], None, u["pb"] * rq)
+    sc = f16n_scale(T)
+    return (T.astype(np.float64) * sc).astype(np.float32), np.float32(1.0 / sc)
+
+
 def _ec_frags(u: Dict[str, np.ndarray], nconv: int) -> np.ndarray:
     return np.concatenate([frag_pack(u[f"G{t}"]).reshape(-1) for t in range(1, nconv + 1)])
 
@@ -356,8 +392,9 @@
     for i in range(2):
         parts = [ec4_weights(units[i], 4, 16)]
         if i == 0:
-            rp, rq, _ = ec4_scales(4, 16, 32)
-            parts.append(frag_pack_f16n(_etab_dense(units[0]["PA"] * rq[:, None], units[0]["QB"] * rq[:, None], None, units[0]["pb"] * rq)))
+            tab, inv_tab = ec1n_unit0_table(units[0])
+            parts.append(_etab_frag1(tab))
+            parts.append(_pad_vec(np.array([inv_tab], np.float32), 64))
         ec1n.append(B.add(np.concatenate(parts)))
     out["ec1n_w"] = ec1n + [None] * (NUM_BLOCKS - 2)
     out["ec_mode"] = ec_mode
@@ -405,24 +442,25 @@
         b6r[4 * q:4 * q + 4] = ip["w_b6"][:4]
     ec = ip["ec"]
     ft = ip["f_tab"]
-    def grp(*mats):
+    def grp(*mats, tables=0):
         sc = min(f16n_scale(m) for m in mats)
-        return sc, [frag_pack_f16n((m.astype(np.float64) * sc).astype(np.float32)) for m in mats]
+        return sc, [(_etab_frag1 if i < tables else frag_pack_f16n)((m.astype(np.float64) * sc).astype(np.float32))
+                    for i, m in enumerate(mats)]
     dtab_d = _etab_dense(ip["d_PA"], ip["d_QB"], ip["d_wn"], ip["d_b0"])
     ectab_d = _etab_dense(ec["PA"][:128], ec["QB"][:128], None, ec["pb"][:128])
     w1tab_d = _etab_dense(ft[:, 0:3], ft[:, 3:6], None, ft[:, 6] + ip["f_b0"])
-    s_dt, (i_dt,) = grp(dtab_d)
+    s_dt, (i_dt,) = grp(dtab_d, tables=1)
     s_d3, (i_d3,) = grp(ip["d_W3"])
-    s_w1, (i_w1t, i_d6, i_w0) = grp(w1tab_d, ip["f_dW"], ip["f_eW"])
+    s_w1, (i_w1t, i_d6, i_w0) = grp(w1tab_d, ip["f_dW"], ip["f_eW"], tables=1)
     ecG = [ec[f"G{t}"] for t in range(1, 8)]
-    s_ec, ec_imgs = grp(ectab_d, *ecG)
+    s_ec, ec_imgs = grp(ectab_d, *ecG, tables=1)
     s_w3, (i_w3,) = grp(ip["w_W3"])
     s_w6, (i_w6r, i_w6f) = grp(W6r, ip["w_W6"])
     io = {}
     for k, im in (("dtab", i_dt), ("ectab", ec_imgs[0]), ("w_b0", i_w1t), ("d_W3", i_d3), ("ec_w", np.concatenate(ec_imgs[1:])),
                   ("d_W6", i_d6), ("w_W3", i_w3)):
         io[k] = B.add(im)
-    assert B.n - io["dtab"] == 76 * 512
+    assert B.n - io["dtab"] == 66 * 512
     io.update({
         "d_b3": B.add(ip["d_b3"] * s_d3),
         "scales": B.add(_pad_vec(np.array([1 / s_dt, 1 / s_d3, 1 / s_w1, 1 / s_ec, 1 / s_w3, 1 / s_w6], np.float32), 16)),
```

Result: faster. 27720 patches/s (median of 6 runs) (+2.2%).
